# mttga/purejaxql

Measured on NVIDIA H100. Metric: MinAtar-Breakout env steps/sec @4096 envs x128 seeds, higher is better.
Workload: dtype f32

## Files before the change

### include/pqn_b200.h

```cpp
#ifndef PQN_B200_H
#define PQN_B200_H

#include <stdint.h>

#ifdef __cplusplus
extern "C" {
#endif

#define PQN_OK 0
#define PQN_E_INVALID (-1)
#define PQN_E_CUDA (-2)
#define PQN_E_UNSUPPORTED (-3)

#define PQN_ENV_BREAKOUT 0
#define PQN_ENV_ASTERIX 1
#define PQN_ENV_SPACE_INVADERS 2
#define PQN_ENV_FREEWAY 3
#define PQN_ENV_SEAQUEST 4
#define PQN_ENV_CARTPOLE 16
#define PQN_ENV_ACROBOT 17
#define PQN_ENV_MOUNTAIN_CAR 18
#define PQN_ENV_MEMORY_CHAIN 32
#define PQN_ENV_CATCH 33
#define PQN_ENV_DEEP_SEA 34
// ... 58 lines not shown
int pqn_rollout_act_step(int env_id, const uint32_t* step_keys, const float* q, const float* eps,
                         uint32_t* state, void* obs_next, int64_t obs_seed_stride, int32_t* action,
                         float* reward, uint8_t* done, float* maxq, int64_t tr_seed_stride, double* info_sums,
                         int info_done_only, int32_t S, int32_t E, int32_t env_total, int32_t env_offset, int max_steps,
                         float rew_scale, int rng_mode, void* stream);
int pqn_rollout_keys(uint32_t* rng_inout, uint32_t* keys_out, int32_t S, int32_t T, int rng_mode, void* stream);

int pqn_qlambda(const float* reward, const uint8_t* done, const float* maxq, const float* q_last,
                float* targets, int32_t T, int32_t S, int32_t E, int32_t A, float gamma, float lambda,
                void* stream);

#define PQN_NET_MINATAR_CNN 0
#define PQN_NET_MLP 1
#define PQN_NET_RNN 2
#define PQN_NET_MLP_BITS 3

typedef struct pqn_net_desc_t {
  int32_t kind;
  int32_t in_c;
  int32_t hidden;
  int32_t layers;
  int32_t num_actions;
  int32_t norm_type;
  int32_t norm_input;
} pqn_net_desc_t;
#define PQN_MAX_LAYERS 8
#define PQN_NORM_LAYER 0
#define PQN_NORM_BATCH 1
#define PQN_NORM_NONE 2

typedef struct pqn_net_layout_t {
  int64_t total;
  int64_t bn_scale, bn_bias;
  int64_t conv_w, conv_b;
  int64_t ln0_scale, ln0_bias;
  int64_t d0_w, d0_b;
  int64_t ln1_scale, ln1_bias;
  int64_t d1_w, d1_b;
  int64_t head_w, head_b;
  int64_t gru_ir_w, gru_ir_b, gru_iz_w, gru_iz_b, gru_in_w, gru_in_b, gru_hr_w, gru_hz_w, gru_hn_w, gru_hn_b;
} pqn_net_layout_t;

int pqn_net_layout(const pqn_net_desc_t* desc_host, pqn_net_layout_t* out_host);
int pqn_net_dense_layer(const pqn_net_desc_t* desc_host, int32_t layer, int64_t* offsets_host);
int64_t pqn_net_stats_floats(const pqn_net_desc_t* desc_host);
int64_t pqn_net_workspace_bytes(const pqn_net_desc_t* desc_host, int32_t S, int64_t rows);

int pqn_net_init(const pqn_net_desc_t* desc_host, const uint32_t* keys, float* params, int32_t S, void* stream);

int pqn_qnet_forward(const pqn_net_desc_t* desc_host, const float* params, const float* batch_stats, const void* obs,
                     const int32_t* gather, int64_t obs_rows_per_seed, float* q, int32_t S, int64_t rows,
                     void* workspace, void* stream);

int pqn_qnet_loss_grad(const pqn_net_desc_t* desc_host, const float* params, float* batch_stats, const void* obs,
                       const int32_t* gather, int64_t obs_rows_per_seed, const int32_t* action,
                       const float* target, int64_t tr_rows_per_seed, float* grads, float* loss_sum,
                       float* qsa_sum, float* bn_sums, int32_t S, int64_t rows, void* workspace, void* stream);

int pqn_rnn_step(const pqn_net_desc_t* desc_host, const float* params, float* hs, const float* obs,
                 int64_t obs_rows_per_seed, const uint8_t* last_done, const int32_t* last_action, float* q, int32_t S,
                 int32_t E, void* workspace, void* stream);
int pqn_rnn_loss_grad(const pqn_net_desc_t* desc_host, const float* params, const float* hs0, const float* obs,
                      const uint8_t* last_done, const int32_t* last_action, const int32_t* action, const float* reward,
                      const uint8_t* done, float* grads, float* loss_sum, float* qsa_sum, int32_t S, int32_t T, int32_t B,
                      float gamma, float lambda, void* workspace, void* stream);
int pqn_rnn_step_stats(const pqn_net_desc_t* desc_host, const float* params, const float* batch_stats, float* hs,
                       const float* obs, int64_t obs_rows_per_seed, const uint8_t* last_done, const int32_t* last_action,
                       float* q, int32_t S, int32_t E, void* workspace, void* stream);
int pqn_rnn_loss_grad_stats(const pqn_net_desc_t* desc_host, const float* params, float* batch_stats, const float* hs0,
                            const float* obs, const uint8_t* last_done, const int32_t* last_action,
                            const int32_t* action, const float* reward, const uint8_t* done, float* grads,
                            float* loss_sum, float* qsa_sum, int32_t S, int32_t T, int32_t B, float gamma, float lambda,
                            void* workspace, void* stream);

int pqn_radam_clip_step(float* params, const float* grads, float* mu, float* nu, const float* sched,
                        int32_t* step_counter, float* gnorm_scratch , int32_t S, int64_t P,
                        float max_norm, float b1, float b2, float eps, void* stream);

int pqn_bn_stats_update(float* batch_stats, float* bn_sums, int32_t S, int32_t F, int64_t stats_seed_stride,
                        float count, float momentum, void* stream);

int pqn_set_tensor_core_path(int on);
int pqn_set_conv_mma_path(int on);

int pqn_tc_split_lo(const float* x, float* lo, int64_t n, void* stream);
int pqn_tc_gemm_test(const float* a, const float* a_lo, const float* b, const float* b_lo, float* d, int32_t S,
                     int32_t M, int32_t N, int32_t K, int a_mn, int b_mn, int split3, void* stream);

int pqn_tc_split16(const float* x, void* hi, void* lo, int64_t n, float scale, void* stream);
int pqn_tc_gemm16_test(const void* a_hi, const void* a_lo, const void* b_hi, const void* b_lo, float* d, int32_t S,
                       int32_t M, int32_t N, int32_t K, int a_mn, int b_mn, float out_scale, void* stream);
int pqn_tc_dgrad16_test(const void* a_hi, const void* a_lo, const void* b_hi, const void* b_lo, const float* mask,
                        const uint32_t* relu_bits, float* d, int32_t S, int32_t M, int32_t N, int32_t K, int epi,
                        float out_scale, void* stream);

#ifdef __cplusplus
}
#endif
#endif
```

### purejaxql_b200/_lib.py

```python
from __future__ import annotations

import ctypes
import os
from ctypes import POINTER, Structure, c_char_p, c_double, c_float, c_int, c_int32, c_int64, c_longlong, c_void_p

HERE = os.path.dirname(os.path.abspath(__file__))
LIB_PATH = os.path.join(HERE, "libpqn_b200.so")


class EnvInfo(Structure):
    _fields_ = [("state_words", c_int32), ("obs_dim", c_int32), ("obs_shape", c_int32 * 3),
                ("num_actions", c_int32), ("max_steps", c_int32), ("binary_obs", c_int32),
                ("packed_obs_words", c_int32)]


class EnvParams(Structure):
    _fields_ = [("max_steps", c_int32), ("memory_length", c_int32)]


class NetDesc(Structure):
    _fields_ = [("kind", c_int32), ("in_c", c_int32), ("hidden", c_int32), ("layers", c_int32),
                ("num_actions", c_int32), ("norm_type", c_int32), ("norm_input", c_int32)]


NORM_TYPES = {"layer_norm": 0, "batch_norm": 1}


class NetLayout(Structure):
    _fields_ = [(n, c_int64) for n in (
        "total", "bn_scale", "bn_bias", "conv_w", "conv_b", "ln0_scale", "ln0_bias", "d0_w", "d0_b",
        "ln1_scale", "ln1_bias", "d1_w", "d1_b", "head_w", "head_b",
        "gru_ir_w", "gru_ir_b", "gru_iz_w", "gru_iz_b", "gru_in_w", "gru_in_b", "gru_hr_w", "gru_hz_w", "gru_hn_w",
        "gru_hn_b")]


class PqnError(RuntimeError):
    pass


_SIGS = {
    "pqn_last_error": (c_char_p, []),
    "pqn_version": (c_int, []),
    "pqn_launch_count": (c_longlong, []),
    "pqn_num_kernels": (c_int, []),
    "pqn_kernel_name": (c_char_p, [c_int]),
    "pqn_profile_enable": (c_int, [c_int]),
    "pqn_profile_read": (c_int, [POINTER(c_double), POINTER(c_longlong), c_int]),
    "pqn_env_info": (c_int, [c_int, POINTER(EnvInfo)]),
    "pqn_rng_split": (c_int, [c_void_p, c_int64, c_int32, c_void_p, c_int, c_void_p]),
    "pqn_threefry2x32": (c_int, [c_void_p, c_void_p, c_void_p, c_int64, c_void_p]),
    "pqn_rng_bits": (c_int, [c_void_p, c_int64, c_int64, c_void_p, c_int, c_void_p]),
    "pqn_random_normal": (c_int, [c_void_p, c_void_p, c_int64, c_int, c_void_p]),
    "pqn_normal_from_bits": (c_int, [c_void_p, c_void_p, c_int64, c_void_p]),
    "pqn_set_permutation_bucket_log2": (c_int, [c_int]),
    "pqn_permutation_workspace_bytes": (c_int64, [c_int64, c_int]),
    "pqn_permutation": (c_int, [c_void_p, c_int64, c_int, c_int, c_void_p, c_int64, c_void_p, c_void_p]),
    "pqn_env_reset": (c_int, [c_int, c_void_p, c_void_p, c_void_p, c_int64, c_int, c_int, c_void_p]),
    "pqn_env_reset_params": (c_int, [c_int, c_void_p, c_void_p, c_void_p, c_int64, POINTER(EnvParams), c_int, c_void_p]),
    "pqn_env_step": (c_int, [c_int, c_void_p, c_void_p, c_void_p, c_void_p, c_void_p, c_void_p, c_void_p,
                             c_void_p, c_void_p, c_void_p, c_int64, c_int, c_int, c_void_p]),
    "pqn_env_obs_packed": (c_int, [c_int, c_void_p, c_void_p, c_int64, c_void_p]),
    "pqn_env_obs": (c_int, [c_int, c_void_p, c_void_p, c_int64, c_void_p]),
    "pqn_eps_greedy": (c_int, [c_void_p, c_void_p, c_void_p, c_void_p, c_int64, c_int32, c_int, c_void_p]),
    "pqn_rollout_act_step": (c_int, [c_int, c_void_p, c_void_p, c_void_p, c_void_p, c_void_p, c_int64, c_void_p,
                                     c_void_p, c_void_p, c_void_p, c_int64, c_void_p, c_int, c_int32, c_int32,
                                     c_int32, c_int32, c_int, c_float, c_int, c_void_p]),
    "pqn_rollout_keys": (c_int, [c_void_p, c_void_p, c_int32, c_int32, c_int, c_void_p]),
    "pqn_qlambda": (c_int, [c_void_p, c_void_p, c_void_p, c_void_p, c_void_p, c_int32, c_int32, c_int32, c_int32,
                            c_float, c_float, c_void_p]),
    "pqn_net_layout": (c_int, [POINTER(NetDesc), POINTER(NetLayout)]),
    "pqn_net_dense_layer": (c_int, [POINTER(NetDesc), c_int32, POINTER(c_int64)]),
    "pqn_net_stats_floats": (c_int64, [POINTER(NetDesc)]),
    "pqn_net_workspace_bytes": (c_int64, [POINTER(NetDesc), c_int32, c_int64]),
    "pqn_net_init": (c_int, [POINTER(NetDesc), c_void_p, c_void_p, c_int32, c_void_p]),
    "pqn_qnet_forward": (c_int, [POINTER(NetDesc), c_void_p, c_void_p, c_void_p, c_void_p, c_int64, c_void_p, c_int32,
                                 c_int64, c_void_p, c_void_p]),
    "pqn_qnet_loss_grad": (c_int, [POINTER(NetDesc), c_void_p, c_void_p, c_void_p, c_void_p, c_int64, c_void_p,
                                   c_void_p, c_int64, c_void_p, c_void_p, c_void_p, c_void_p, c_int32, c_int64,
                                   c_void_p, c_void_p]),
    "pqn_rnn_step": (c_int, [POINTER(NetDesc), c_void_p, c_void_p, c_void_p, c_int64, c_void_p, c_void_p, c_void_p,
                             c_int32, c_int32, c_void_p, c_void_p]),
    "pqn_rnn_loss_grad": (c_int, [POINTER(NetDesc), c_void_p, c_void_p, c_void_p, c_void_p, c_void_p, c_void_p, c_void_p,
                                  c_void_p, c_void_p, c_void_p, c_void_p, c_int32, c_int32, c_int32, c_float, c_float,
                                  c_void_p, c_void_p]),
    "pqn_rnn_step_stats": (c_int, [POINTER(NetDesc), c_void_p, c_void_p, c_void_p, c_void_p, c_int64, c_void_p, c_void_p,
                                   c_void_p, c_int32, c_int32, c_void_p, c_void_p]),
    "pqn_rnn_loss_grad_stats": (c_int, [POINTER(NetDesc), c_void_p, c_void_p, c_void_p, c_void_p, c_void_p, c_void_p,
                                        c_void_p, c_void_p, c_void_p, c_void_p, c_void_p, c_void_p, c_int32, c_int32,
                                        c_int32, c_float, c_float, c_void_p, c_void_p]),
    "pqn_radam_clip_step": (c_int, [c_void_p, c_void_p, c_void_p, c_void_p, c_void_p, c_void_p, c_void_p, c_int32,
                                    c_int64, c_float, c_float, c_float, c_float, c_void_p]),
    "pqn_bn_stats_update": (c_int, [c_void_p, c_void_p, c_int32, c_int32, c_int64, c_float, c_float, c_void_p]),
    "pqn_set_tensor_core_path": (c_int, [c_int]),
    "pqn_set_conv_mma_path": (c_int, [c_int]),
    "pqn_tc_split_lo": (c_int, [c_void_p, c_void_p, c_int64, c_void_p]),
    "pqn_tc_split16": (c_int, [c_void_p, c_void_p, c_void_p, c_int64, c_float, c_void_p]),
    "pqn_tc_gemm_test": (c_int, [c_void_p, c_void_p, c_void_p, c_void_p, c_void_p, c_int32, c_int32, c_int32,
                                 c_int32, c_int, c_int, c_int, c_void_p]),
    "pqn_tc_gemm16_test": (c_int, [c_void_p, c_void_p, c_void_p, c_void_p, c_void_p, c_int32, c_int32, c_int32,
                                   c_int32, c_int, c_int, c_float, c_void_p]),
    "pqn_tc_dgrad16_test": (c_int, [c_void_p, c_void_p, c_void_p, c_void_p, c_void_p, c_void_p, c_void_p, c_int32,
                                    c_int32, c_int32, c_int32, c_int, c_float, c_void_p]),
}

EXPORTS = tuple(_SIGS)
_lib = None


def lib():
    global _lib
    if _lib is None:
        if not os.path.exists(LIB_PATH):
            raise PqnError(
                f"{LIB_PATH} is not built. Run `python -m purejaxql_b200.build` (needs nvcc). "
                "purejaxql_b200 has no CPU fallback.")
        l = ctypes.CDLL(LIB_PATH)
        for name, (res, args) in _SIGS.items():
            fn = getattr(l, name)
            fn.restype = res
            fn.argtypes = args
        _lib = l
    return _lib


def check(rc: int, what: str = ""):
    if rc != 0:
        msg = lib().pqn_last_error().decode("utf-8", "replace")
        raise PqnError(f"{what or 'libpqn_b200'} failed (rc={rc}): {msg}")


def p(t):
    if t is None:
        return None
    if not t.is_cuda:
        raise PqnError("libpqn_b200 takes CUDA tensors only (no CPU fallback); got a CPU tensor")
    if not t.is_contiguous():
        raise PqnError("libpqn_b200 takes contiguous tensors")
    return c_void_p(t.data_ptr())


def raw(t):
    if t is None:
        return None
    if not t.is_cuda:
        raise PqnError("libpqn_b200 takes CUDA tensors only (no CPU fallback); got a CPU tensor")
    return c_void_p(t.data_ptr())


def stream_ptr():
    import torch
    return c_void_p(torch.cuda.current_stream().cuda_stream)


def profile_read(reset=True):
    l = lib()
    n = l.pqn_num_kernels()
    ms = (c_double * n)()
    cnt = (c_longlong * n)()
    check(l.pqn_profile_read(ms, cnt, 1 if reset else 0), "pqn_profile_read")
    return {l.pqn_kernel_name(i).decode(): (ms[i], int(cnt[i])) for i in range(n) if cnt[i]}
```

### purejaxql_b200/csrc/pqn_net.cu

```cuda
#include <cuda_runtime.h>
#include <stdint.h>

#include "../../include/pqn_b200.h"
#include "api_common.h"
#include "tc_common.cuh"

namespace pqn {

constexpr int GT = 256;
constexpr int BK = 16;
constexpr float LN_EPS = 1e-6f;
constexpr int CONV_O = 16;
constexpr int CONV_PIX = 64;
constexpr int HID_CNN = 128;
constexpr int FLAT_CNN = CONV_PIX * CONV_O;

static int g_use_tc = 2;
static int g_conv_mma = 1;

__host__ __device__ static inline int64_t align4(int64_t x) { return (x + 3) & ~(int64_t)3; }

static int make_layout(const pqn_net_desc_t* d, pqn_net_layout_t* L) {
  int64_t off = 0;
  auto take = [&](int64_t n) { int64_t o = off; off += align4(n); return o; };
  L->d1_w = L->d1_b = L->ln1_scale = L->ln1_bias = L->conv_w = L->conv_b = -1;
  L->gru_ir_w = L->gru_ir_b = L->gru_iz_w = L->gru_iz_b = L->gru_in_w = L->gru_in_b = -1;
  L->gru_hr_w = L->gru_hz_w = L->gru_hn_w = L->gru_hn_b = -1;
  const int A = d->num_actions;
  const bool has_norm = d->norm_type != PQN_NORM_NONE;
  if (d->kind == PQN_NET_MINATAR_CNN) {
    const int C = d->in_c;
    L->bn_scale = take(C); L->bn_bias = take(C);
    L->conv_w = take(9 * C * CONV_O); L->conv_b = take(CONV_O);
    L->ln0_scale = L->ln0_bias = -1;
    if (has_norm) { L->ln0_scale = take(CONV_O); L->ln0_bias = take(CONV_O); }
    L->d0_w = take((int64_t)FLAT_CNN * HID_CNN); L->d0_b = take(HID_CNN);
    if (has_norm) { L->ln1_scale = take(HID_CNN); L->ln1_bias = take(HID_CNN); }
    L->head_w = take((int64_t)HID_CNN * A); L->head_b = take(A);
  } else if (d->kind == PQN_NET_MLP || d->kind == PQN_NET_RNN || d->kind == PQN_NET_MLP_BITS) {
    const int D = d->in_c, H = d->hidden;
    L->bn_scale = take(D); L->bn_bias = take(D);
    L->d0_w = take((int64_t)D * H); L->d0_b = take(H);
    L->ln0_scale = L->ln0_bias = -1;
    if (has_norm) { L->ln0_scale = take(H); L->ln0_bias = take(H); }
    for (int l = 1; l < d->layers; ++l) {
      const int64_t w = take((int64_t)H * H), b = take(H);
      const int64_t sc = has_norm ? take(H) : -1, bi = has_norm ? take(H) : -1;
      if (l == 1) { L->d1_w = w; L->d1_b = b; L->ln1_scale = sc; L->ln1_bias = bi; }
    }
    if (d->kind == PQN_NET_RNN) {
      L->gru_ir_w = take((int64_t)(H + A) * H); L->gru_ir_b = take(H);
      L->gru_iz_w = take((int64_t)(H + A) * H); L->gru_iz_b = take(H);
      L->gru_in_w = take((int64_t)(H + A) * H); L->gru_in_b = take(H);
      L->gru_hr_w = take((int64_t)H * H); L->gru_hz_w = take((int64_t)H * H);
      L->gru_hn_w = take((int64_t)H * H); L->gru_hn_b = take(H);
    }
    L->head_w = take((int64_t)H * A); L->head_b = take(A);
  } else {
    return -1;
  }
  L->total = off;
  return 0;
}

struct DenseOff { int64_t w, b, g, bi; };
__host__ __device__ inline DenseOff dense_off(const pqn_net_layout_t& L, int H, int l) {
  if (l == 0) return DenseOff{L.d0_w, L.d0_b, L.ln0_scale, L.ln0_bias};
  if (l == 1) return DenseOff{L.d1_w, L.d1_b, L.ln1_scale, L.ln1_bias};
  const bool norm = L.ln1_scale >= 0;
  const int64_t stride = align4((int64_t)H * H) + (norm ? 3 : 1) * align4(H);
  const int64_t w = (norm ? L.ln1_bias : L.d1_b) + align4(H) + (l - 2) * stride;
  const int64_t b = w + align4((int64_t)H * H);
  return DenseOff{w, b, norm ? b + align4(H) : -1, norm ? b + 2 * align4(H) : -1};
}

static int check_desc(const pqn_net_desc_t* d, const char* who) {
  if (!d) return set_error(PQN_E_INVALID, "%s: desc is NULL", who);
  if (d->num_actions < 1 || d->num_actions > 32) return set_error(PQN_E_INVALID, "%s: num_actions=%d out of [1,32]", who, d->num_actions);
  if (d->norm_type < 0 || d->norm_type > 2 || d->norm_input < 0 || d->norm_input > 1)
    return set_error(PQN_E_INVALID, "%s: norm_type=%d norm_input=%d", who, d->norm_type, d->norm_input);
  if (d->kind == PQN_NET_MLP || d->kind == PQN_NET_RNN || d->kind == PQN_NET_MLP_BITS) {
    const int H = d->hidden;
    if (H != 64 && H != 128 && H != 256 && H != 512)
      return set_error(PQN_E_UNSUPPORTED, "%s: hidden=%d (64, 128, 256 or 512 built)", who, H);
    if (d->layers < 1 || d->layers > PQN_MAX_LAYERS)
      return set_error(PQN_E_UNSUPPORTED, "%s: layers=%d (1 to %d built)", who, d->layers, PQN_MAX_LAYERS);
  }
  {
    const int Nh = d->kind == PQN_NET_MINATAR_CNN ? 128 : d->hidden;
    const size_t need = (size_t)(24 * Nh + 9 * d->num_actions * Nh + 8 * d->num_actions + 16) * sizeof(float);
    if (need > 227u * 1024u)
      return set_error(PQN_E_UNSUPPORTED, "%s: hidden=%d with num_actions=%d needs %zu B of shared memory for the head "
                       "backward (limit 227 KB)", who, Nh, d->num_actions, need);
  }
  if (d->kind == PQN_NET_MINATAR_CNN) {
    if (d->in_c != 4 && d->in_c != 6 && d->in_c != 7 && d->in_c != 10)
      return set_error(PQN_E_UNSUPPORTED, "%s: CNN in_c=%d (MinAtar uses 4/6/7/10)", who, d->in_c);
    return PQN_OK;
  }
  if (d->kind == PQN_NET_MLP_BITS) {
    if (d->in_c != 400 && d->in_c != 600 && d->in_c != 700)
// ... 494 lines not shown
      if (DZLO != nullptr) {
        float lo[V];
#pragma unroll
        for (int k = 0; k < V; ++k) lo[k] = tc::tf32_lo(dz[V * c + k]);
        st_feat<V>(DZLO + e, lo);
      }
    }
  }
#pragma unroll
  for (int j = 0; j < F; ++j) {
    const int f = (j / V) * CW + lane * V + (j % V);
    s_red3[warp * 3 * N + f] = a_dsc[j];
    s_red3[warp * 3 * N + N + f] = a_dbi[j];
    s_red3[warp * 3 * N + 2 * N + f] = a_db[j];
  }
  if (HEAD && lane == 0) { s_ls[warp * 2] = a_loss; s_ls[warp * 2 + 1] = a_qsa; }
  __syncthreads();
  const int stride = 3 * N + (HEAD ? A * N + A + 2 : 0);
  float* __restrict__ o = part + ((int64_t)seed * gridDim.x + blockIdx.x) * stride;
  for (int i = tid; i < 3 * N; i += 256) {
    float v = 0.f;
#pragma unroll
    for (int wv = 0; wv < 8; ++wv) v += s_red3[wv * 3 * N + i];
    o[i] = v;
  }
  if (HEAD) {
    for (int i = tid; i < A * N; i += 256) {
      float v = 0.f;
#pragma unroll
      for (int wv = 0; wv < 8; ++wv) v += s_dhw[wv * A * N + i];
      o[3 * N + i] = v;
    }
    if (tid < A + 2) {
      float v = 0.f;
      for (int wv = 0; wv < 8; ++wv) v += tid < A ? s_dhb[wv * A + tid] : s_ls[wv * 2 + (tid - A)];
      o[3 * N + A * N + tid] = v;
    }
  }
}

template <int SL>
__device__ __forceinline__ float ordered_partial_sum(const float* __restrict__ p, int count, int64_t stride, bool valid) {
  constexpr int COLS = 256 / SL;
  __shared__ float slice_sum[SL][COLS];
  const int col = threadIdx.x % COLS, sl = threadIdx.x / COLS;
  float v = 0.f;
  if (valid) {
#pragma unroll 4
    for (int c = sl; c < count; c += SL) v += p[(int64_t)c * stride];
  }
  slice_sum[sl][col] = v;
  __syncthreads();
  float r = 0.f;
  if (sl == 0) {
#pragma unroll
    for (int k = 0; k < SL; ++k) r += slice_sum[k][col];
  }
  return r;
}
static inline int final_slices(int count) { return count > 48 ? 32 : 8; }

template <int SL>
__global__ void row_bwd_final_kernel(const float* __restrict__ part, int nctas, int N, int A, int head,
                                     float* __restrict__ grads, int64_t P, int64_t off_dscale, int64_t off_dbias,
                                     int64_t off_db, int64_t off_hw, int64_t off_hb, float* __restrict__ loss_sum,
                                     float* __restrict__ qsa_sum) {
  const int seed = blockIdx.y;
  const int stride = 3 * N + (head ? A * N + A + 2 : 0);
  const int i = blockIdx.x * (256 / SL) + threadIdx.x % (256 / SL);
  const float v = ordered_partial_sum<SL>(part + (int64_t)seed * nctas * stride + i, nctas, stride, i < stride);
  if (i >= stride || threadIdx.x >= 256 / SL) return;
  float* __restrict__ g = grads + (int64_t)seed * P;
  if (i < N) g[off_dscale + i] = v;
  else if (i < 2 * N) g[off_dbias + (i - N)] = v;
  else if (i < 3 * N) g[off_db + (i - 2 * N)] = v;
  else if (i < 3 * N + A * N) {
    const int j = i - 3 * N, a = j / N, f = j - a * N;
    g[off_hw + (int64_t)f * A + a] = v;
  } else if (i < 3 * N + A * N + A) g[off_hb + (i - 3 * N - A * N)] = v;
  else if (i == 3 * N + A * N + A) loss_sum[seed] += v;
  else qsa_sum[seed] += v;
}

template <int C>
struct ConvCfg {
  static constexpr int TAPS = 9 * C;
  static constexpr int OBS_BITS = 100 * C;
  static constexpr int OBS_WORDS = (OBS_BITS + 31) / 32;
  static constexpr int PW = (OBS_WORDS + 3) / 4 * 4;
  static constexpr int SW = PW + 1;
};

template <int C>
__device__ __forceinline__ uint32_t pixel_bits(const uint32_t* __restrict__ so, int p) {
  const int f0 = p * C;
  const uint32_t lo = so[f0 >> 5], hi = so[(f0 >> 5) + 1];
  return __funnelshift_r(lo, hi, f0 & 31) & ((1u << C) - 1u);
}

template <int C>
__device__ __forceinline__ void conv_pixel(const uint32_t* __restrict__ so, const float* __restrict__ ws,
                                           const float* __restrict__ cb, int y, int x, float (&acc)[CONV_O]) {
#pragma unroll
  for (int o = 0; o < CONV_O; ++o) acc[o] = cb[o];
#pragma unroll
  for (int di = 0; di < 3; ++di)
#pragma unroll
    for (int dj = 0; dj < 3; ++dj) {
      const uint32_t nib = pixel_bits<C>(so, (y + di) * 10 + (x + dj));
      if (__ballot_sync(0xffffffffu, nib != 0u) == 0u) continue;
#pragma unroll
      for (int c = 0; c < C; ++c) {
        const bool bit = (nib >> c) & 1u;
        if (__ballot_sync(0xffffffffu, bit) == 0u) continue;
        const float* __restrict__ w = ws + ((di * 3 + dj) * C + c) * CONV_O;
#pragma unroll
        for (int o4 = 0; o4 < CONV_O / 4; ++o4) {
          const float4 wv = *reinterpret_cast<const float4*>(w + 4 * o4);
          if (bit) {
            acc[4 * o4] += wv.x; acc[4 * o4 + 1] += wv.y; acc[4 * o4 + 2] += wv.z; acc[4 * o4 + 3] += wv.w;
          }
        }
      }
    }
}

__device__ __forceinline__ void ln16(const float (&z)[CONV_O], float& mean, float& rstd) {
  float s1 = 0.f, s2 = 0.f;
#pragma unroll
  for (int o = 0; o < CONV_O; ++o) { s1 += z[o]; s2 = fmaf(z[o], z[o], s2); }
  mean = s1 * (1.0f / CONV_O);
  const float var = fmaxf(s2 * (1.0f / CONV_O) - mean * mean, 0.f);
  rstd = 1.0f / sqrtf(var + LN_EPS);
}

template <int C>
__device__ __forceinline__ void conv_load_consts(const float* __restrict__ prm, const pqn_net_layout_t& L, float* ws,
                                                 float* cb, float* sc, float* bi) {
  const float inv255 = 1.0f / 255.0f;
  for (int i = threadIdx.x; i < ConvCfg<C>::TAPS * CONV_O; i += blockDim.x) ws[i] = __ldg(prm + L.conv_w + i) * inv255;
  if (threadIdx.x < CONV_O) {
    cb[threadIdx.x] = __ldg(prm + L.conv_b + threadIdx.x);
    sc[threadIdx.x] = __ldg(prm + L.ln0_scale + threadIdx.x);
    bi[threadIdx.x] = __ldg(prm + L.ln0_bias + threadIdx.x);
  }
}

template <int C, bool TRAIN>
__global__ void __launch_bounds__(256) conv_fwd_kernel(const uint32_t* __restrict__ obs, int64_t obs_rows_per_seed,
                                                       const int32_t* __restrict__ gather,
                                                       const float* __restrict__ params, int64_t P,
                                                       pqn_net_layout_t L, float* __restrict__ H1,
                                                       float* __restrict__ H1LO, float* __restrict__ bn_sums,
                                                       int rows) {
  using Cfg = ConvCfg<C>;
  __shared__ __align__(16) float ws[Cfg::TAPS * CONV_O];
  __shared__ float cb[CONV_O], sc[CONV_O], bi[CONV_O];
  __shared__ uint32_t so[4][Cfg::SW];
  __shared__ float s_cnt[C];
  const int tid = threadIdx.x, sl = tid >> 6, pix = tid & 63;
  const int seed = blockIdx.y;
  const int row = blockIdx.x * 4 + sl;
  const bool valid = row < rows;
  conv_load_consts<C>(params + (int64_t)seed * P, L, ws, cb, sc, bi);
  if (TRAIN && tid < C) s_cnt[tid] = 0.f;
  if (pix < Cfg::SW) {
    uint32_t w = 0u;
    if (valid && pix < Cfg::PW) {
      const int64_t src = gather ? gather[(int64_t)seed * rows + row] : row;
      w = __ldg(obs + ((int64_t)seed * obs_rows_per_seed + src) * Cfg::PW + pix);
    }
    so[sl][pix] = w;
  }
  __syncthreads();
// ... 121 lines not shown
        float4 dz;
        dz.x = rstd * (dy[4 * o4] - m1 - acc[4 * o4] * m2);
        dz.y = rstd * (dy[4 * o4 + 1] - m1 - acc[4 * o4 + 1] * m2);
        dz.z = rstd * (dy[4 * o4 + 2] - m1 - acc[4 * o4 + 2] * m2);
        dz.w = rstd * (dy[4 * o4 + 3] - m1 - acc[4 * o4 + 3] * m2);
        *reinterpret_cast<float4*>(&my_dz[pix * SDZ_LD + 4 * o4]) = dz;
      }
    }
    __syncwarp();
#pragma unroll 8
    for (int p = tpar; p < CONV_PIX; p += 2) a_dcb += my_dz[p * SDZ_LD + o_b];
#pragma unroll
    for (int c = 0; c < C; ++c) {
      for (int wi = 0; wi < Cfg::OBS_WORDS; ++wi) {
        uint32_t bits = my_so[wi];
        if (C == 4) bits &= 0x11111111u << c;
        if (bits == 0u) continue;
        while (bits) {
          const int b = __ffs(bits) - 1;
          bits &= bits - 1u;
          const int f = wi * 32 + b;
          const int q = f / C;
          if (f - q * C != c) continue;
          const int qy = q / 10, qx = q - qy * 10;
#pragma unroll
          for (int it = 0; it < 5; ++it) {
            const int py = qy - t_di[it], px = qx - t_dj[it];
            if ((unsigned)py < 8u && (unsigned)px < 8u) wacc[c][it] += my_dz[(py * 8 + px) * SDZ_LD + o_b];
          }
        }
      }
    }
  }
  __syncthreads();
  for (int i = tid; i < TAPS * CONV_O; i += blockDim.x) s_w[i] = 0.f;
  __syncthreads();
  const float inv255 = 1.0f / 255.0f;
#pragma unroll
  for (int c = 0; c < C; ++c)
#pragma unroll
    for (int it = 0; it < 5; ++it) {
      const int tap = it * 2 + tpar;
      if (tap < 9) atomicAdd(&s_w[(tap * C + c) * CONV_O + o_b], wacc[c][it] * inv255);
    }
  atomicAdd(&s_red[2 * CONV_O + o_b], a_dcb);
#pragma unroll
  for (int o = 0; o < CONV_O; ++o) {
    float v0 = a_dsc[o], v1 = a_dbi[o];
#pragma unroll
    for (int sft = 16; sft > 0; sft >>= 1) {
      v0 += __shfl_xor_sync(0xffffffffu, v0, sft);
      v1 += __shfl_xor_sync(0xffffffffu, v1, sft);
    }
    if (lane == 0) {
      atomicAdd(&s_red[o], v0);
      atomicAdd(&s_red[CONV_O + o], v1);
    }
  }
  __syncthreads();
  float* __restrict__ g = grads + (int64_t)seed * P;
  for (int i = tid; i < TAPS * CONV_O; i += blockDim.x) atomicAdd(g + L.conv_w + i, s_w[i]);
  if (tid < CONV_O) {
    atomicAdd(g + L.ln0_scale + tid, s_red[tid]);
    atomicAdd(g + L.ln0_bias + tid, s_red[CONV_O + tid]);
    atomicAdd(g + L.conv_b + tid, s_red[2 * CONV_O + tid]);
  }
}

__device__ __forceinline__ void mma_tf32_16n8k8(float (&d)[4], const uint32_t (&a)[4], uint32_t b0, uint32_t b1) {
  asm volatile(
      "mma.sync.aligned.m16n8k8.row.col.f32.tf32.tf32.f32 {%0,%1,%2,%3}, {%4,%5,%6,%7}, {%8,%9}, {%0,%1,%2,%3};"
      : "+f"(d[0]), "+f"(d[1]), "+f"(d[2]), "+f"(d[3])
      : "r"(a[0]), "r"(a[1]), "r"(a[2]), "r"(a[3]), "r"(b0), "r"(b1));
}

template <int C>
struct ConvMma {
  static constexpr int TAPS = 9 * C;
  static constexpr int KS = (TAPS + 7) / 8;
  static constexpr int MT = (TAPS + 15) / 16;
};

template <int C>
struct PatchCfg {
  static constexpr int WORDS = (9 * C + 31) / 32;
};

template <int C>
__device__ __forceinline__ void patch_bits(const uint32_t* __restrict__ so, int pix, uint32_t (&w)[PatchCfg<C>::WORDS]) {
  constexpr int W = PatchCfg<C>::WORDS;
#pragma unroll
  for (int k = 0; k < W; ++k) w[k] = 0u;
  const int y = pix >> 3, x = pix & 7;
#pragma unroll
  for (int di = 0; di < 3; ++di) {
    const int f0 = ((y + di) * 10 + x) * C;
    const uint32_t r = __funnelshift_r(so[f0 >> 5], so[(f0 >> 5) + 1], f0 & 31) & ((1u << (3 * C)) - 1u);
    const int o = 3 * C * di;
    w[o >> 5] |= r << (o & 31);
    if ((o & 31) + 3 * C > 32) w[min((o >> 5) + 1, W - 1)] |= r >> (32 - (o & 31));
  }
}

template <int C>
__device__ __forceinline__ void build_patch(const uint32_t* __restrict__ so, int pix, uint32_t* __restrict__ out) {
  constexpr int W = PatchCfg<C>::WORDS;
  uint32_t w[W];
  patch_bits<C>(so, pix, w);
#pragma unroll
  for (int k = 0; k < W; ++k) out[k] = w[k];
}

template <int C>
__device__ __forceinline__ void build_patches(const uint32_t* __restrict__ so, uint32_t* __restrict__ patch, int lane) {
  build_patch<C>(so, lane, patch + lane * PatchCfg<C>::WORDS);
  build_patch<C>(so, lane + 32, patch + (lane + 32) * PatchCfg<C>::WORDS);
}

__device__ __forceinline__ uint32_t bit_f32(uint32_t word, int shift) {
  return ((word >> shift) & 1u) ? 0x3F800000u : 0u;
}

template <int C, bool EXPC = false>
__device__ __forceinline__ void conv_mma_load_weights(const float* __restrict__ prm, const pqn_net_layout_t& L,
                                                      float2* wb_hi, float2* wb_lo, float* cb, float* sc, float* bi) {
  using M = ConvMma<C>;
  const float inv255 = 1.0f / 255.0f;
  for (int i = threadIdx.x; i < M::KS * 2 * 32; i += blockDim.x) {
    const int ln = i & 31, h = (i >> 5) & 1, ks = i >> 6;
    const int o = h * 8 + (ln >> 2);
    const int t0 = ks * 8 + (ln & 3), t1 = t0 + 4;
    float w0 = t0 < M::TAPS ? __ldg(prm + L.conv_w + t0 * CONV_O + o) * inv255 : 0.f;
    float w1 = t1 < M::TAPS ? __ldg(prm + L.conv_w + t1 * CONV_O + o) * inv255 : 0.f;
    if (EXPC) {
      w0 *= __uint_as_float((254u - (1u << (t0 & 7))) << 23);
      w1 *= __uint_as_float((254u - (1u << (t1 & 7))) << 23);
    }
    const float h0 = __uint_as_float(__float_as_uint(w0) & 0xFFFFE000u), h1 = __uint_as_float(__float_as_uint(w1) & 0xFFFFE000u);
    wb_hi[i] = make_float2(h0, h1);
    wb_lo[i] = make_float2(w0 - h0, w1 - h1);
  }
  if (threadIdx.x < CONV_O) {
    cb[threadIdx.x] = __ldg(prm + L.conv_b + threadIdx.x);
    sc[threadIdx.x] = __ldg(prm + L.ln0_scale + threadIdx.x);
    bi[threadIdx.x] = __ldg(prm + L.ln0_bias + threadIdx.x);
  }
}

template <int C>
struct ExpPatch {
  static constexpr int KS = ConvMma<C>::KS;
  static constexpr int LD = KS | 1;
};

template <int C>
__device__ __forceinline__ void build_exp_patch(const uint32_t* __restrict__ so, int pix, uint32_t* __restrict__ out) {
  constexpr int W = PatchCfg<C>::WORDS;
  uint32_t w[W];
  patch_bits<C>(so, pix, w);
#pragma unroll
  for (int ks = 0; ks < ExpPatch<C>::KS; ++ks)
    out[ks] = ((w[(8 * ks) >> 5] >> ((8 * ks) & 31)) & 0xFFu) << 23;
}

template <int C>
__device__ __forceinline__ void conv_mma_block2_exp(const uint32_t* __restrict__ xp, const float2* __restrict__ wb_hi,
                                                    const float2* __restrict__ wb_lo, const float* __restrict__ cb,
                                                    int mbp, int lane, float (&z)[2][2][4]) {
  using E = ExpPatch<C>;
  const int g = lane >> 2, t = lane & 3;
  const uint32_t m_lo = 1u << (23 + t), m_hi = 1u << (27 + t);
#pragma unroll
  for (int i = 0; i < 2; ++i)
#pragma unroll
    for (int h = 0; h < 2; ++h) {
      z[i][h][0] = z[i][h][2] = cb[8 * h + 2 * t];
      z[i][h][1] = z[i][h][3] = cb[8 * h + 2 * t + 1];
    }
  const uint32_t* r00 = xp + (32 * mbp + g) * E::LD;
#pragma unroll
  for (int ks = 0; ks < E::KS; ++ks) {
    uint32_t a[2][4];
#pragma unroll
    for (int i = 0; i < 2; ++i) {
      const uint32_t w0 = r00[(16 * i) * E::LD + ks], w1 = r00[(16 * i + 8) * E::LD + ks];
      a[i][0] = w0 & m_lo; a[i][1] = w1 & m_lo; a[i][2] = w0 & m_hi; a[i][3] = w1 & m_hi;
    }
    float2 bl[2], bh[2];
#pragma unroll
    for (int h = 0; h < 2; ++h) {
      bl[h] = wb_lo[(ks * 2 + h) * 32 + lane];
      bh[h] = wb_hi[(ks * 2 + h) * 32 + lane];
    }
#pragma unroll
    for (int h = 0; h < 2; ++h)
#pragma unroll
      for (int i = 0; i < 2; ++i) mma_tf32_16n8k8(z[i][h], a[i], __float_as_uint(bl[h].x), __float_as_uint(bl[h].y));
#pragma unroll
    for (int h = 0; h < 2; ++h)
#pragma unroll
      for (int i = 0; i < 2; ++i) mma_tf32_16n8k8(z[i][h], a[i], __float_as_uint(bh[h].x), __float_as_uint(bh[h].y));
  }
}

__device__ __forceinline__ void ln16_quad(const float (&z)[2][4], float& mean0, float& rstd0, float& mean1,
                                          float& rstd1) {
  float s0 = z[0][0] + z[0][1] + z[1][0] + z[1][1];
  float q0 = z[0][0] * z[0][0] + z[0][1] * z[0][1] + z[1][0] * z[1][0] + z[1][1] * z[1][1];
  float s1 = z[0][2] + z[0][3] + z[1][2] + z[1][3];
  float q1 = z[0][2] * z[0][2] + z[0][3] * z[0][3] + z[1][2] * z[1][2] + z[1][3] * z[1][3];
#pragma unroll
  for (int o = 1; o <= 2; o <<= 1) {
    s0 += __shfl_xor_sync(0xffffffffu, s0, o); q0 += __shfl_xor_sync(0xffffffffu, q0, o);
    s1 += __shfl_xor_sync(0xffffffffu, s1, o); q1 += __shfl_xor_sync(0xffffffffu, q1, o);
  }
  mean0 = s0 * (1.0f / CONV_O); mean1 = s1 * (1.0f / CONV_O);
  rstd0 = rsqrtf(fmaxf(q0 * (1.0f / CONV_O) - mean0 * mean0, 0.f) + LN_EPS);
  rstd1 = rsqrtf(fmaxf(q1 * (1.0f / CONV_O) - mean1 * mean1, 0.f) + LN_EPS);
}

constexpr int CONV_MMA_WARPS = 8;

template <int C, bool TRAIN, bool H16 = false>
__global__ void __launch_bounds__(CONV_MMA_WARPS * 32, 3)
    conv_fwd_mma_kernel(const uint32_t* __restrict__ obs, int64_t obs_rows_per_seed, const int32_t* __restrict__ gather,
                        const float* __restrict__ params, int64_t P, pqn_net_layout_t L, float* __restrict__ H1,
                        float* __restrict__ H1LO, float* __restrict__ XH1, float* __restrict__ RS1,
                        uint32_t* __restrict__ RB, float* __restrict__ bn_sums, int rows) {
  using Cfg = ConvCfg<C>;
  using M = ConvMma<C>;
  __shared__ float2 wb_hi[M::KS * 2 * 32], wb_lo[M::KS * 2 * 32];
  __shared__ float cb[CONV_O], sc[CONV_O], bi[CONV_O];
  __shared__ uint32_t so[CONV_MMA_WARPS][Cfg::SW];
  __shared__ uint32_t sxp[CONV_MMA_WARPS][CONV_PIX * ExpPatch<C>::LD];
  __shared__ float s_cnt[C];
  const int tid = threadIdx.x, warp = tid >> 5, lane = tid & 31;
  const int g = lane >> 2, t = lane & 3;
  const int seed = blockIdx.y;
  conv_mma_load_weights<C, true>(params + (int64_t)seed * P, L, wb_hi, wb_lo, cb, sc, bi);
  if (TRAIN && tid < C) s_cnt[tid] = 0.f;
  __syncthreads();
  int cnt[C];
  uint32_t cmask[C];
#pragma unroll
  for (int c = 0; c < C; ++c) {
    cnt[c] = 0;
    cmask[c] = 0u;
    if (TRAIN) {
      for (int b = 0; b < 32; ++b) {
        const int f = lane * 32 + b;
        if (f < Cfg::OBS_BITS && f % C == c) cmask[c] |= 1u << b;
      }
    }
  }
  uint32_t* __restrict__ my_so = so[warp];
  static_assert(Cfg::PW <= 32, "one packed observation word per lane");
  if (lane == 0) my_so[Cfg::PW] = 0u;
  const int row_stride = gridDim.x * CONV_MMA_WARPS;
  auto fetch = [&](int r) -> uint32_t {
    if (r >= rows || lane >= Cfg::PW) return 0u;
    const int64_t src = gather ? gather[(int64_t)seed * rows + r] : r;
    return __ldg(obs + ((int64_t)seed * obs_rows_per_seed + src) * Cfg::PW + lane);
  };
  uint32_t pre = fetch(blockIdx.x * CONV_MMA_WARPS + warp);
  for (int row = blockIdx.x * CONV_MMA_WARPS + warp; row < rows; row += row_stride) {
    __syncwarp();
    if (lane < Cfg::PW) my_so[lane] = pre;
    if (TRAIN && bn_sums != nullptr) {
#pragma unroll
      for (int c = 0; c < C; ++c) cnt[c] += __popc(pre & cmask[c]);
    }
    __syncwarp();
    pre = fetch(row + row_stride);
    build_exp_patch<C>(my_so, lane, sxp[warp] + lane * ExpPatch<C>::LD);
    build_exp_patch<C>(my_so, lane + 32, sxp[warp] + (lane + 32) * ExpPatch<C>::LD);
    __syncwarp();
    float* __restrict__ hrow = H16 ? nullptr : H1 + ((int64_t)seed * rows + row) * FLAT_CNN;
    float* __restrict__ lrow = (!H16 && H1LO) ? H1LO + ((int64_t)seed * rows + row) * FLAT_CNN : nullptr;
    __half* __restrict__ hrow16 = H16 ? reinterpret_cast<__half*>(H1) + ((int64_t)seed * rows + row) * FLAT_CNN : nullptr;
    __half* __restrict__ lrow16 = H16 ? reinterpret_cast<__half*>(H1LO) + ((int64_t)seed * rows + row) * FLAT_CNN : nullptr;
    float* __restrict__ xrow = (TRAIN && XH1) ? XH1 + ((int64_t)seed * rows + row) * FLAT_CNN : nullptr;
    float* __restrict__ rrow = (TRAIN && RS1) ? RS1 + ((int64_t)seed * rows + row) * CONV_PIX : nullptr;
    uint16_t* __restrict__ brow =
        (TRAIN && RB) ? reinterpret_cast<uint16_t*>(RB + ((int64_t)seed * rows + row) * (FLAT_CNN / 32)) : nullptr;
#pragma unroll 1
    for (int mbp = 0; mbp < 2; ++mbp) {
     float z2[2][2][4];
     conv_mma_block2_exp<C>(sxp[warp], wb_hi, wb_lo, cb, mbp, lane, z2);
#pragma unroll
     for (int mi = 0; mi < 2; ++mi) {
      const int mb = 2 * mbp + mi;
      float (&z)[2][4] = z2[mi];
      float mean0, rstd0, mean1, rstd1;
      ln16_quad(z, mean0, rstd0, mean1, rstd1);
      uint32_t rb0 = 0u, rb1 = 0u;
#pragma unroll
      for (int h = 0; h < 2; ++h) {
        const int o = 8 * h + 2 * t;
        float2 v0, v1;
        v0.x = fmaxf((z[h][0] - mean0) * rstd0 * sc[o] + bi[o], 0.f);
        v0.y = fmaxf((z[h][1] - mean0) * rstd0 * sc[o + 1] + bi[o + 1], 0.f);
        v1.x = fmaxf((z[h][2] - mean1) * rstd1 * sc[o] + bi[o], 0.f);
        v1.y = fmaxf((z[h][3] - mean1) * rstd1 * sc[o + 1] + bi[o + 1], 0.f);
        const int p0 = 16 * mb + g, p1 = p0 + 8;
        if (H16) {
          __half2 h0, l0, h1v, l1;
          tc::split16x2<false>(fminf(v0.x, 65000.f), fminf(v0.y, 65000.f), h0, l0);
          tc::split16x2<false>(fminf(v1.x, 65000.f), fminf(v1.y, 65000.f), h1v, l1);
          *reinterpret_cast<__half2*>(hrow16 + p0 * CONV_O + o) = h0;
          *reinterpret_cast<__half2*>(lrow16 + p0 * CONV_O + o) = l0;
          *reinterpret_cast<__half2*>(hrow16 + p1 * CONV_O + o) = h1v;
          *reinterpret_cast<__half2*>(lrow16 + p1 * CONV_O + o) = l1;
        } else {
          *reinterpret_cast<float2*>(hrow + p0 * CONV_O + o) = v0;
          *reinterpret_cast<float2*>(hrow + p1 * CONV_O + o) = v1;
        }
        if (TRAIN) {
          rb0 |= ((v0.x > 0.f ? 1u : 0u) | (v0.y > 0.f ? 2u : 0u)) << o;
          rb1 |= ((v1.x > 0.f ? 1u : 0u) | (v1.y > 0.f ? 2u : 0u)) << o;
        }
        if (xrow) {
          *reinterpret_cast<float2*>(xrow + p0 * CONV_O + o) =
              make_float2((z[h][0] - mean0) * rstd0, (z[h][1] - mean0) * rstd0);
          *reinterpret_cast<float2*>(xrow + p1 * CONV_O + o) =
              make_float2((z[h][2] - mean1) * rstd1, (z[h][3] - mean1) * rstd1);
          if (h == 0 && t == 0) { rrow[p0] = rstd0; rrow[p1] = rstd1; }
        }
        if (lrow) {
          *reinterpret_cast<float2*>(lrow + p0 * CONV_O + o) = make_float2(tc::tf32_lo(v0.x), tc::tf32_lo(v0.y));
          *reinterpret_cast<float2*>(lrow + p1 * CONV_O + o) = make_float2(tc::tf32_lo(v1.x), tc::tf32_lo(v1.y));
        }
      }
      if (TRAIN && brow) {
        rb0 |= __shfl_xor_sync(0xffffffffu, rb0, 1); rb1 |= __shfl_xor_sync(0xffffffffu, rb1, 1);
        rb0 |= __shfl_xor_sync(0xffffffffu, rb0, 2); rb1 |= __shfl_xor_sync(0xffffffffu, rb1, 2);
        if (t == 0) { brow[16 * mb + g] = (uint16_t)rb0; brow[16 * mb + g + 8] = (uint16_t)rb1; }
      }
     }
    }
  }
  if (TRAIN && bn_sums != nullptr) {
#pragma unroll
    for (int c = 0; c < C; ++c) {
      int v = cnt[c];
#pragma unroll
      for (int o = 16; o > 0; o >>= 1) v += __shfl_xor_sync(0xffffffffu, v, o);
      if (lane == 0 && v) atomicAdd(&s_cnt[c], (float)v);
    }
    __syncthreads();
    if (tid < C && s_cnt[tid] != 0.f) {
      atomicAdd(bn_sums + (int64_t)seed * 2 * C + tid, s_cnt[tid]);
      atomicAdd(bn_sums + (int64_t)seed * 2 * C + C + tid, s_cnt[tid]);
    }
  }
}

__device__ __forceinline__ void mma_f16_16n8k16(float (&d)[4], const uint32_t (&a)[4], uint32_t b0, uint32_t b1) {
  asm volatile(
      "mma.sync.aligned.m16n8k16.row.col.f32.f16.f16.f32 {%0,%1,%2,%3}, {%4,%5,%6,%7}, {%8,%9}, {%0,%1,%2,%3};"
      : "+f"(d[0]), "+f"(d[1]), "+f"(d[2]), "+f"(d[3])
      : "r"(a[0]), "r"(a[1]), "r"(a[2]), "r"(a[3]), "r"(b0), "r"(b1));
}

template <int C>
struct Conv16 {
  static constexpr int TAPS = 9 * C;
  static constexpr int KS = (TAPS + 15) / 16;
  static constexpr int ROW = 2 * KS < 8 ? 8 : 2 * KS;
};

__host__ __device__ constexpr int conv16_channel(int h, int n) { return 4 * (n >> 1) + 2 * h + (n & 1); }

__host__ __device__ constexpr int conv16_tap(int s, int kk) {
  return 16 * s + (kk < 8 ? 0 : 8) + ((kk & 1) ? 4 : 0) + ((kk & 7) >> 1);
}

template <int C>
__device__ __forceinline__ void conv16_load_weights(const float* __restrict__ prm, const pqn_net_layout_t& L, uint4* wb,
                                                    float* cb, float* sc, float* bi) {
  using M = Conv16<C>;
  const float inv255 = 1.0f / 255.0f;
  for (int i = threadIdx.x; i < M::KS * 2 * 32; i += blockDim.x) {
    const int ln = i & 31, h = (i >> 5) & 1, s = i >> 6;
    const int gg = ln >> 2, tt = ln & 3;
    const int o = conv16_channel(h, gg);
    const float scale = __uint_as_float((uint32_t)(127 + 15 - (1 << tt)) << 23);
    float v[4];
#pragma unroll
    for (int q = 0; q < 4; ++q) {
      const int tap = conv16_tap(s, 2 * tt + (q & 1) + (q >> 1) * 8);
      v[q] = tap < M::TAPS ? __ldg(prm + L.conv_w + tap * CONV_O + o) * inv255 * scale : 0.f;
      v[q] = fminf(fmaxf(v[q], -65000.f), 65000.f);
    }
    const __half2 h0 = __floats2half2_rn(v[0], v[1]), h1 = __floats2half2_rn(v[2], v[3]);
    const float2 f0 = __half22float2(h0), f1 = __half22float2(h1);
    const __half2 l0 = __floats2half2_rn(v[0] - f0.x, v[1] - f0.y), l1 = __floats2half2_rn(v[2] - f1.x, v[3] - f1.y);
    wb[i] = make_uint4(*reinterpret_cast<const uint32_t*>(&h0), *reinterpret_cast<const uint32_t*>(&h1),
                       *reinterpret_cast<const uint32_t*>(&l0), *reinterpret_cast<const uint32_t*>(&l1));
  }
  if (threadIdx.x < CONV_O) {
    cb[threadIdx.x] = __ldg(prm + L.conv_b + threadIdx.x);
    sc[threadIdx.x] = __ldg(prm + L.ln0_scale + threadIdx.x);
    bi[threadIdx.x] = __ldg(prm + L.ln0_bias + threadIdx.x);
  }
}

template <int C>
__device__ __forceinline__ void build_patch16(const uint32_t* __restrict__ so, int pix, uint32_t* __restrict__ out) {
  constexpr int W = PatchCfg<C>::WORDS;
  uint32_t w[W];
  patch_bits<C>(so, pix, w);
#pragma unroll
  for (int b = 0; b < 2 * Conv16<C>::KS; ++b) {
    const int o = 8 * b;
    uint32_t v = (o >> 5) < W ? w[(o >> 5) < W ? (o >> 5) : 0] : 0u;
    const int sh = o & 31;
    const uint32_t lo = sh >= 10 ? v >> (sh - 10) : v << (10 - sh);
    const uint32_t hi = sh + 4 <= 26 ? v << (26 - sh - 4) : v >> (sh + 4 - 26);
    out[b] = __byte_perm(lo, hi, 0x7610);
  }
}

template <int C>
__device__ __forceinline__ void store_patch16(const uint32_t* __restrict__ so, int pix, uint32_t* __restrict__ row) {
  using M = Conv16<C>;
  uint32_t w[M::ROW];
#pragma unroll
  for (int k = 0; k < M::ROW; ++k) w[k] = 0u;
  build_patch16<C>(so, pix, w);
#pragma unroll
  for (int q = 0; q < M::ROW / 4; ++q)
    *reinterpret_cast<uint4*>(row + 4 * q) = make_uint4(w[4 * q], w[4 * q + 1], w[4 * q + 2], w[4 * q + 3]);
}

template <int C>
__device__ __forceinline__ void conv16_block2(const uint32_t* __restrict__ xp, const uint4* __restrict__ wb,
                                              const float* __restrict__ cb, int mbp, int lane, float (&z)[2][2][4]) {
  using M = Conv16<C>;
  const int g = lane >> 2, t = lane & 3;
  const uint32_t mask = (1u << (10 + t)) | (1u << (26 + t));
#pragma unroll
  for (int i = 0; i < 2; ++i)
#pragma unroll
    for (int h = 0; h < 2; ++h) {
      z[i][h][0] = z[i][h][2] = cb[4 * t + 2 * h];
      z[i][h][1] = z[i][h][3] = cb[4 * t + 2 * h + 1];
    }
  const uint32_t* r00 = xp + (32 * mbp + g) * M::ROW;
#pragma unroll
  for (int s = 0; s < M::KS; ++s) {
    uint32_t a[2][4];
#pragma unroll
    for (int i = 0; i < 2; ++i) {
      const uint2 w0 = *reinterpret_cast<const uint2*>(r00 + (16 * i) * M::ROW + 2 * s);
      const uint2 w1 = *reinterpret_cast<const uint2*>(r00 + (16 * i + 8) * M::ROW + 2 * s);
      a[i][0] = w0.x & mask; a[i][1] = w1.x & mask; a[i][2] = w0.y & mask; a[i][3] = w1.y & mask;
    }
    uint4 b[2];
#pragma unroll
    for (int h = 0; h < 2; ++h) b[h] = wb[(s * 2 + h) * 32 + lane];
#pragma unroll
    for (int h = 0; h < 2; ++h)
#pragma unroll
      for (int i = 0; i < 2; ++i) mma_f16_16n8k16(z[i][h], a[i], b[h].z, b[h].w);
#pragma unroll
    for (int h = 0; h < 2; ++h)
#pragma unroll
      for (int i = 0; i < 2; ++i) mma_f16_16n8k16(z[i][h], a[i], b[h].x, b[h].y);
  }
}

__device__ __forceinline__ uint32_t cvt_f16x2_satfinite(float lo, float hi) {
  uint32_t r;
  asm("cvt.rn.satfinite.f16x2.f32 %0, %1, %2;" : "=r"(r) : "f"(hi), "f"(lo));
  return r;
}

constexpr int CONV16_WARPS = 4;
constexpr int CONV16_CTAS_PER_SM = 5;

template <int C, bool TRAIN, bool H16>
__global__ void __launch_bounds__(CONV16_WARPS * 32, CONV16_CTAS_PER_SM)
    conv_fwd_mma16_kernel(const uint32_t* __restrict__ obs, int64_t obs_rows_per_seed, const int32_t* __restrict__ gather,
                          const float* __restrict__ params, int64_t P, pqn_net_layout_t L, float* __restrict__ H1,
                          float* __restrict__ H1LO, float* __restrict__ XH1, float* __restrict__ RS1,
                          uint32_t* __restrict__ RB, float* __restrict__ bn_sums, int rows) {
  using Cfg = ConvCfg<C>;
  using M = Conv16<C>;
  __shared__ __align__(16) uint4 wb[M::KS * 2 * 32];
  __shared__ float cb[CONV_O], sc[CONV_O], bi[CONV_O];
  __shared__ uint32_t so[CONV16_WARPS][Cfg::SW];
  __shared__ __align__(16) uint32_t sxp[CONV16_WARPS][CONV_PIX * M::ROW];
  __shared__ float s_cnt[C];
  const int tid = threadIdx.x, warp = tid >> 5, lane = tid & 31;
  const int g = lane >> 2, t = lane & 3;
  const int seed = blockIdx.y;
  conv16_load_weights<C>(params + (int64_t)seed * P, L, wb, cb, sc, bi);
  if (TRAIN && tid < C) s_cnt[tid] = 0.f;
  __syncthreads();
  int cnt[C];
  uint32_t cmask[C];
#pragma unroll
  for (int c = 0; c < C; ++c) {
    cnt[c] = 0;
    cmask[c] = 0u;
    if (TRAIN) {
      for (int b = 0; b < 32; ++b) {
        const int f = lane * 32 + b;
        if (f < Cfg::OBS_BITS && f % C == c) cmask[c] |= 1u << b;
      }
    }
  }
  uint32_t* __restrict__ my_so = so[warp];
  static_assert(Cfg::PW <= 32, "one packed observation word per lane");
  if (lane == 0) my_so[Cfg::PW] = 0u;
  const int row_stride = gridDim.x * CONV16_WARPS;
  auto fetch_index = [&](int r) -> int {
    const int rc = r < rows ? r : rows - 1;
    return gather ? __ldg(gather + (int64_t)seed * rows + rc) : rc;
  };
  auto fetch_obs = [&](int src) -> uint32_t {
    return __ldg(obs + ((int64_t)seed * obs_rows_per_seed + src) * Cfg::PW + (lane < Cfg::PW ? lane : 0));
  };
  const int row0 = blockIdx.x * CONV16_WARPS + warp;
  uint32_t pre = fetch_obs(fetch_index(row0));
  int src_next = fetch_index(row0 + row_stride);
  for (int row = row0; row < rows; row += row_stride) {
    __syncwarp();
    if (lane < Cfg::PW) my_so[lane] = pre;
    if (TRAIN && bn_sums != nullptr) {
#pragma unroll
      for (int c = 0; c < C; ++c) cnt[c] += __popc(pre & cmask[c]);
    }
    __syncwarp();
    pre = fetch_obs(src_next);
    src_next = fetch_index(row + 2 * row_stride);
    store_patch16<C>(my_so, lane, sxp[warp] + lane * M::ROW);
    store_patch16<C>(my_so, lane + 32, sxp[warp] + (lane + 32) * M::ROW);
    __syncwarp();
    const int64_t grow = (int64_t)seed * rows + row;
    float* __restrict__ hrow = H16 ? nullptr : H1 + grow * FLAT_CNN;
    __half* __restrict__ hrow16 = H16 ? reinterpret_cast<__half*>(H1) + grow * FLAT_CNN : nullptr;
    __half* __restrict__ lrow16 = H16 ? reinterpret_cast<__half*>(H1LO) + grow * FLAT_CNN : nullptr;
    float* __restrict__ xrow = (TRAIN && XH1) ? XH1 + grow * FLAT_CNN : nullptr;
    float* __restrict__ rrow = (TRAIN && RS1) ? RS1 + grow * CONV_PIX : nullptr;
    uint16_t* __restrict__ brow = (TRAIN && RB) ? reinterpret_cast<uint16_t*>(RB + grow * (FLAT_CNN / 32)) : nullptr;
    float keep_rs0 = 0.f, keep_rs1 = 0.f;
    uint32_t keep_rb = 0u;
#pragma unroll 1
    for (int mbp = 0; mbp < 2; ++mbp) {
      float z2[2][2][4];
      conv16_block2<C>(sxp[warp], wb, cb, mbp, lane, z2);
#pragma unroll
      for (int mi = 0; mi < 2; ++mi) {
        const int mb = 2 * mbp + mi;
        float (&z)[2][4] = z2[mi];
        float mean0, rstd0, mean1, rstd1;
        ln16_quad(z, mean0, rstd0, mean1, rstd1);
        const float nm0 = -mean0 * rstd0, nm1 = -mean1 * rstd1;
        uint32_t rb0 = 0u, rb1 = 0u;
        const int p0 = 16 * mb + g, p1 = p0 + 8, o4 = 4 * t;
        float x0[4], x1[4], v0[4], v1[4];
#pragma unroll
        for (int h = 0; h < 2; ++h) {
#pragma unroll
          for (int c = 0; c < 2; ++c) {
            const int o = o4 + 2 * h + c;
            x0[2 * h + c] = fmaf(z[h][c], rstd0, nm0);
            x1[2 * h + c] = fmaf(z[h][2 + c], rstd1, nm1);
            v0[2 * h + c] = fmaxf(fmaf(x0[2 * h + c], sc[o], bi[o]), 0.f);
            v1[2 * h + c] = fmaxf(fmaf(x1[2 * h + c], sc[o], bi[o]), 0.f);
          }
        }
        if (H16) {
          uint32_t hw0[2], hw1[2], lw0[2], lw1[2];
#pragma unroll
          for (int h = 0; h < 2; ++h) {
            hw0[h] = cvt_f16x2_satfinite(v0[2 * h], v0[2 * h + 1]);
            hw1[h] = cvt_f16x2_satfinite(v1[2 * h], v1[2 * h + 1]);
            const float2 f0 = __half22float2(*reinterpret_cast<const __half2*>(&hw0[h]));
// ... 922 lines not shown
  switch (C) {
    case 4: { LaunchScope _ls(TRAIN ? K_CONV_FWD : K_CONV_FWD_INFER, st); conv_fwd_kernel<4, TRAIN><<<grid, 256, 0, st>>>(obs, orps, gather, params, P, L, h1, h1lo, bn, rows); } break;
    case 6: { LaunchScope _ls(TRAIN ? K_CONV_FWD : K_CONV_FWD_INFER, st); conv_fwd_kernel<6, TRAIN><<<grid, 256, 0, st>>>(obs, orps, gather, params, P, L, h1, h1lo, bn, rows); } break;
    case 7: { LaunchScope _ls(TRAIN ? K_CONV_FWD : K_CONV_FWD_INFER, st); conv_fwd_kernel<7, TRAIN><<<grid, 256, 0, st>>>(obs, orps, gather, params, P, L, h1, h1lo, bn, rows); } break;
    case 10: { LaunchScope _ls(TRAIN ? K_CONV_FWD : K_CONV_FWD_INFER, st); conv_fwd_kernel<10, TRAIN><<<grid, 256, 0, st>>>(obs, orps, gather, params, P, L, h1, h1lo, bn, rows); } break;
    default: return -1;
  }
  return 0;
}

static unsigned conv_bwd_ctas(int S, int rows) {
  int per_seed = (device_sm_count() * 2 * 4 + S - 1) / S;
  const int maxc = (rows + CONV_BWD_WARPS - 1) / CONV_BWD_WARPS;
  if (per_seed > maxc) per_seed = maxc;
  if (per_seed < 1) per_seed = 1;
  return (unsigned)per_seed;
}

static int wgrad_splits(int tiles, int S, int rows) {
  int s = (2 * device_sm_count() + tiles * S - 1) / (tiles * S);
  const int maxs = (rows + 255) / 256;
  if (s > maxs) s = maxs;
  if (s < 1) s = 1;
  return s;
}

__global__ void split_lo_strided_kernel(const float* __restrict__ src, int64_t src_seed_stride, float* __restrict__ lo,
                                        int64_t n_per_seed) {
  const int seed = blockIdx.y;
  const int64_t i4 = (int64_t)blockIdx.x * blockDim.x + threadIdx.x;
  if (i4 * 4 >= n_per_seed) return;
  const float4 v = __ldg(reinterpret_cast<const float4*>(src + (int64_t)seed * src_seed_stride) + i4);
  reinterpret_cast<float4*>(lo + (int64_t)seed * n_per_seed)[i4] =
      make_float4(tc::tf32_lo(v.x), tc::tf32_lo(v.y), tc::tf32_lo(v.z), tc::tf32_lo(v.w));
}

static void launch_split_w1(const float* params, int64_t P, int64_t off_w, float* w1_lo, int S, cudaStream_t st) {
  const int64_t n = (int64_t)FLAT_CNN * HID_CNN;
  LaunchScope _ls(K_TC_SPLIT, st);
  split_lo_strided_kernel<<<dim3(cdiv(n / 4, 256), S), 256, 0, st>>>(params + off_w, P, w1_lo, n);
}

struct Planes16 { __half *h1_hi, *h1_lo, *dz_hi, *dz_lo, *w1_hi, *w1_lo; };
static Planes16 planes16(const Workspace& w, int S, int64_t rows) {
  const int64_t R = (int64_t)S * rows;
  Planes16 p;
  p.h1_hi = reinterpret_cast<__half*>(w.h1_lo); p.h1_lo = p.h1_hi + R * FLAT_CNN;
  p.dz_hi = reinterpret_cast<__half*>(w.dz2_lo); p.dz_lo = p.dz_hi + R * HID_CNN;
  p.w1_hi = reinterpret_cast<__half*>(w.w1_lo); p.w1_lo = p.w1_hi + (int64_t)S * FLAT_CNN * HID_CNN;
  return p;
}
static float grad_scale(int64_t rows) {
  float s = 16.f;
  while (rows > 1) { s *= 2.f; rows = (rows + 1) >> 1; }
  return s;
}

__global__ void split16_strided_kernel(const float* __restrict__ src, int64_t src_seed_stride, __half* __restrict__ hi,
                                       __half* __restrict__ lo, int64_t n_per_seed) {
  const int seed = blockIdx.y;
  const int64_t i4 = (int64_t)blockIdx.x * blockDim.x + threadIdx.x;
  if (i4 * 4 >= n_per_seed) return;
  const float4 v = __ldg(reinterpret_cast<const float4*>(src + (int64_t)seed * src_seed_stride) + i4);
  __half2 h0, h1, l0, l1;
  tc::split16x2(v.x, v.y, h0, l0);
  tc::split16x2(v.z, v.w, h1, l1);
  reinterpret_cast<uint2*>(hi + (int64_t)seed * n_per_seed)[i4] =
      make_uint2(*reinterpret_cast<uint32_t*>(&h0), *reinterpret_cast<uint32_t*>(&h1));
  reinterpret_cast<uint2*>(lo + (int64_t)seed * n_per_seed)[i4] =
      make_uint2(*reinterpret_cast<uint32_t*>(&l0), *reinterpret_cast<uint32_t*>(&l1));
}

static void launch_split16_w1(const float* params, int64_t P, int64_t off_w, const Planes16& pl, int S, cudaStream_t st) {
  const int64_t n = (int64_t)FLAT_CNN * HID_CNN;
  LaunchScope _ls(K_TC_SPLIT, st);
  split16_strided_kernel<<<dim3(cdiv(n / 4, 256), S), 256, 0, st>>>(params + off_w, P, pl.w1_hi, pl.w1_lo, n);
}
static void launch_split16_h1(const float* h1, const Planes16& pl, int64_t n, cudaStream_t st) {
  LaunchScope _ls(K_TC_SPLIT, st);
  split16_strided_kernel<<<dim3(cdiv(n / 4, 256), 1), 256, 0, st>>>(h1, 0, pl.h1_hi, pl.h1_lo, n);
}

static int tc16_dense_fwd(int epi, const float* params, int64_t P, const pqn_net_layout_t& L, const Workspace& w,
                          const Planes16& pl, int A, float* q, int S, int rows, cudaStream_t st) {
  CUtensorMap t[4];
  int rc;
  if ((rc = tc::make_tmap16(&t[0], pl.h1_hi, FLAT_CNN, rows, S, FLAT_CNN, (uint64_t)rows * FLAT_CNN, 128))) return rc;
  if ((rc = tc::make_tmap16(&t[1], pl.h1_lo, FLAT_CNN, rows, S, FLAT_CNN, (uint64_t)rows * FLAT_CNN, 128))) return rc;
  if ((rc = tc::make_tmap16(&t[2], pl.w1_hi, HID_CNN, FLAT_CNN, S, HID_CNN, (uint64_t)FLAT_CNN * HID_CNN, 64))) return rc;
  if ((rc = tc::make_tmap16(&t[3], pl.w1_lo, HID_CNN, FLAT_CNN, S, HID_CNN, (uint64_t)FLAT_CNN * HID_CNN, 64))) return rc;
  tc::GemmShape gs = {};
  gs.S = S; gs.M = rows; gs.m_tiles = (rows + 127) / 128; gs.n_tiles = 1; gs.k_blocks = FLAT_CNN / tc::TC_BK16;
  tc::EpiParams ep = {};
  ep.params = params; ep.P = P; ep.off_b = L.d0_b; ep.off_scale = L.ln1_scale; ep.off_bias = L.ln1_bias;
  ep.off_hw = L.head_w; ep.off_hb = L.head_b; ep.A = A; ep.rows = rows;
  ep.H = w.h2; ep.XHAT = w.xhat2; ep.RSTD = w.rstd2; ep.Q = q;
  return tc::launch_gemm16(0, 1, epi, t, gs, ep, st, epi == tc::EPI_LN_HEAD ? K_TC_FWD_HEAD : K_TC_FWD);
}

static int tc16_wgrad(float* grads, int64_t P, const pqn_net_layout_t& L, const Planes16& pl, int S, int rows,
                      float gscale, float* wg_part, cudaStream_t st) {
  CUtensorMap t[4];
  int rc;
  if ((rc = tc::make_tmap16(&t[0], pl.h1_hi, FLAT_CNN, rows, S, FLAT_CNN, (uint64_t)rows * FLAT_CNN, 64))) return rc;
  if ((rc = tc::make_tmap16(&t[1], pl.h1_lo, FLAT_CNN, rows, S, FLAT_CNN, (uint64_t)rows * FLAT_CNN, 64))) return rc;
  if ((rc = tc::make_tmap16(&t[2], pl.dz_hi, HID_CNN, rows, S, HID_CNN, (uint64_t)rows * HID_CNN, 64))) return rc;
  if ((rc = tc::make_tmap16(&t[3], pl.dz_lo, HID_CNN, rows, S, HID_CNN, (uint64_t)rows * HID_CNN, 64))) return rc;
  tc::GemmShape gs = {};
  gs.S = S; gs.M = FLAT_CNN; gs.m_tiles = FLAT_CNN / 128; gs.n_tiles = 1;
  gs.k_blocks = (rows + tc::TC_BK16 - 1) / tc::TC_BK16;
  gs.k_split = wgrad_ksplit(S * gs.m_tiles * gs.n_tiles, gs.k_blocks);
  tc::EpiParams ep = {};
  ep.ld_out = HID_CNN; ep.out_scale = 1.0f / gscale;
  const int64_t n = (int64_t)FLAT_CNN * HID_CNN;
  if (gs.k_split > 1) { ep.out = wg_part; ep.out_seed_stride = n; ep.split_stride = (int64_t)S * n; }
  else { ep.out = grads + L.d0_w; ep.out_seed_stride = P; }
  if ((rc = tc::launch_gemm16(1, 1, tc::EPI_STORE, t, gs, ep, st, K_TC_WGRAD))) return rc;
  if (gs.k_split > 1) {
    launch_split_reduce(wg_part, gs.k_split, (int64_t)S * n, n, S, grads + L.d0_w, P, st);
  }
  return 0;
}

static int tc16_dgrad(const Workspace& w, const Planes16& pl, int S, int rows, bool have_bits, float gscale,
                      cudaStream_t st) {
  CUtensorMap t[4];
  int rc;
  if ((rc = tc::make_tmap16(&t[0], pl.dz_hi, HID_CNN, rows, S, HID_CNN, (uint64_t)rows * HID_CNN, 128))) return rc;
  if ((rc = tc::make_tmap16(&t[1], pl.dz_lo, HID_CNN, rows, S, HID_CNN, (uint64_t)rows * HID_CNN, 128))) return rc;
  if ((rc = tc::make_tmap16(&t[2], pl.w1_hi, HID_CNN, FLAT_CNN, S, HID_CNN, (uint64_t)FLAT_CNN * HID_CNN, 128))) return rc;
  if ((rc = tc::make_tmap16(&t[3], pl.w1_lo, HID_CNN, FLAT_CNN, S, HID_CNN, (uint64_t)FLAT_CNN * HID_CNN, 128))) return rc;
  tc::GemmShape gs = {};
  gs.S = S; gs.M = rows; gs.m_tiles = (rows + 127) / 128; gs.n_tiles = FLAT_CNN / 128; gs.k_blocks = HID_CNN / tc::TC_BK16;
 
  tc::EpiParams ep = {};
  ep.out = w.h1; ep.mask = w.h1; ep.ld_out = FLAT_CNN; ep.out_seed_stride = (int64_t)rows * FLAT_CNN;
  ep.relu_bits = w.relu_bits; ep.rows = rows; ep.out_scale = 1.0f / gscale;
  return tc::launch_gemm16(0, 0, have_bits ? tc::EPI_RELU_BITS : tc::EPI_RELU_MASK, t, gs, ep, st, K_TC_DGRAD);
}

static int tc16_mm_store(const __half* a, int64_t a_plane, const __half* b, int64_t b_plane, float* out, int S, int rows, int K,
                         int N, cudaStream_t st, int kid) {
  CUtensorMap t[4];
  int rc;
  if ((rc = tc::make_tmap16(&t[0], a, K, rows, S, K, (uint64_t)rows * K, 128))) return rc;
  if ((rc = tc::make_tmap16(&t[1], a + a_plane, K, rows, S, K, (uint64_t)rows * K, 128))) return rc;
  if ((rc = tc::make_tmap16(&t[2], b, N, K, S, N, (uint64_t)K * N, 64))) return rc;
  if ((rc = tc::make_tmap16(&t[3], b + b_plane, N, K, S, N, (uint64_t)K * N, 64))) return rc;
  tc::GemmShape gs = {};
  gs.S = S; gs.M = rows; gs.m_tiles = (rows + 127) / 128; gs.n_tiles = N / 128; gs.k_blocks = (K + tc::TC_BK16 - 1) / tc::TC_BK16;
 
  tc::EpiParams ep = {};
  ep.out = out; ep.ld_out = N; ep.out_seed_stride = (int64_t)rows * N;
  return tc::launch_gemm16(0, 1, tc::EPI_STORE, t, gs, ep, st, kid);
}
static int tc16_mm_wgrad(const __half* a, int64_t a_plane, const __half* dz, int64_t dz_plane, float* out, int64_t out_seed_stride,
                         int S, int rows, int M, int N, float out_scale, float* wg_part, cudaStream_t st) {
  CUtensorMap t[4];
  int rc;
  if ((rc = tc::make_tmap16(&t[0], a, M, rows, S, M, (uint64_t)rows * M, 64))) return rc;
  if ((rc = tc::make_tmap16(&t[1], a + a_plane, M, rows, S, M, (uint64_t)rows * M, 64))) return rc;
  if ((rc = tc::make_tmap16(&t[2], dz, N, rows, S, N, (uint64_t)rows * N, 64))) return rc;
  if ((rc = tc::make_tmap16(&t[3], dz + dz_plane, N, rows, S, N, (uint64_t)rows * N, 64))) return rc;
  tc::GemmShape gs = {};
  gs.S = S; gs.M = M; gs.m_tiles = M / 128; gs.n_tiles = N / 128; gs.k_blocks = (rows + tc::TC_BK16 - 1) / tc::TC_BK16;
  gs.k_split = wgrad_ksplit(S * gs.m_tiles * gs.n_tiles, gs.k_blocks);
  tc::EpiParams ep = {};
  ep.ld_out = N; ep.out_scale = out_scale;
  const int64_t n = (int64_t)M * N;
  if (gs.k_split > 1) { ep.out = wg_part; ep.out_seed_stride = n; ep.split_stride = (int64_t)S * n; }
  else { ep.out = out; ep.out_seed_stride = out_seed_stride; }
  if ((rc = tc::launch_gemm16(1, 1, tc::EPI_STORE, t, gs, ep, st, K_TC_WGRAD))) return rc;
  if (gs.k_split > 1) {
    launch_split_reduce(wg_part, gs.k_split, (int64_t)S * n, n, S, out, out_seed_stride, st);
  }
  return 0;
}
static int tc16_mm_dgrad(const __half* dz, int64_t dz_plane, const __half* wgt, int64_t w_plane, const float* mask, float* out,
                         int S, int rows, int N, int Kp, float out_scale, cudaStream_t st) {
// ... 224 lines not shown
  if (rnn::modular_rnn(d)) {
    if ((rc = rnn::rnn_trunk_bwd_modular(d, L, params, obs, grads, S, rows, w, st))) return rc;
    return check_launch(who);
  }
  const dim3 rbg(conv_mma_ctas(S, rows, 4), S);
  float* dcur = w.dx;
  for (int l = d->layers - 1; l >= 0; --l) {
    const DenseOff o = dense_off(L, H, l);
    if ((rc = run_row_bwd(H, false, rbg, A, st, nullptr, w.xh[l], w.rs[l], dcur, dcur, nullptr, nullptr, nullptr, 1.0f, params,
                          grads, P, o.g, o.bi, o.b, 0, 0, nullptr, nullptr, nullptr, 0, nullptr, nullptr, w.rbp,
                          rows))) return rc;
    const float* xprev = l == 0 ? obs : w.h[l - 1];
    const int kin = l == 0 ? D : H;
    const int spl = wgrad_splits(ffma_tiles(kin, H), S, rows);
    run_wgrad_ffma(xprev, (int64_t)rows * kin, kin, dcur, (int64_t)rows * H, H, grads, P, o.w, rows, kin, S, spl, w.wgp, st);
    if (l > 0) {
      float* dnext = dcur == w.dhl ? w.dx : w.dhl;
      launch_dgrad(dcur, (int64_t)rows * H, H, params, P, o.w, w.h[l - 1], dnext, (int64_t)rows * H, rows, H, 0, S, st);
      dcur = dnext;
    }
  }
  return check_launch(who);
}

}

using namespace pqn;

extern "C" {

int64_t pqn_net_stats_floats(const pqn_net_desc_t* d) {
  if (check_desc(d, "pqn_net_stats_floats")) return -1;
  return nrm::stats_floats(d);
}

int pqn_rnn_step(const pqn_net_desc_t* d, const float* params, float* hs, const float* obs, int64_t obs_rows_per_seed,
                 const uint8_t* last_done, const int32_t* last_action, float* q, int32_t S, int32_t E, void* workspace,
                 void* stream) {
  int rc = check_desc(d, "pqn_rnn_step");
  if (rc) return rc;
  if ((rc = rnn::check_rnn(d, "pqn_rnn_step"))) return rc;
  return rnn_step(d, params, nullptr, hs, obs, obs_rows_per_seed, last_done, last_action, q, S, E, workspace, stream,
                  "pqn_rnn_step");
}

int pqn_rnn_step_stats(const pqn_net_desc_t* d, const float* params, const float* batch_stats, float* hs, const float* obs,
                       int64_t obs_rows_per_seed, const uint8_t* last_done, const int32_t* last_action, float* q, int32_t S,
                       int32_t E, void* workspace, void* stream) {
  int rc = check_desc(d, "pqn_rnn_step_stats");
  if (rc) return rc;
  if ((rc = rnn::check_rnn_stats(d, batch_stats, "pqn_rnn_step_stats"))) return rc;
  return rnn_step(d, params, batch_stats, hs, obs, obs_rows_per_seed, last_done, last_action, q, S, E, workspace, stream,
                  "pqn_rnn_step_stats");
}

int pqn_rnn_loss_grad(const pqn_net_desc_t* d, const float* params, const float* hs0, const float* obs,
                      const uint8_t* last_done, const int32_t* last_action, const int32_t* action, const float* reward,
                      const uint8_t* done, float* grads, float* loss_sum, float* qsa_sum, int32_t S, int32_t T, int32_t B,
                      float gamma, float lambda, void* workspace, void* stream) {
  int rc = check_desc(d, "pqn_rnn_loss_grad");
  if (rc) return rc;
  if ((rc = rnn::check_rnn(d, "pqn_rnn_loss_grad"))) return rc;
  return rnn_loss_grad(d, params, nullptr, hs0, obs, last_done, last_action, action, reward, done, grads, loss_sum, qsa_sum,
                       S, T, B, gamma, lambda, workspace, stream, "pqn_rnn_loss_grad");
}

int pqn_rnn_loss_grad_stats(const pqn_net_desc_t* d, const float* params, float* batch_stats, const float* hs0,
                            const float* obs, const uint8_t* last_done, const int32_t* last_action, const int32_t* action,
                            const float* reward, const uint8_t* done, float* grads, float* loss_sum, float* qsa_sum,
                            int32_t S, int32_t T, int32_t B, float gamma, float lambda, void* workspace, void* stream) {
  int rc = check_desc(d, "pqn_rnn_loss_grad_stats");
  if (rc) return rc;
  if ((rc = rnn::check_rnn_stats(d, batch_stats, "pqn_rnn_loss_grad_stats"))) return rc;
  return rnn_loss_grad(d, params, batch_stats, hs0, obs, last_done, last_action, action, reward, done, grads, loss_sum,
                       qsa_sum, S, T, B, gamma, lambda, workspace, stream, "pqn_rnn_loss_grad_stats");
}

int pqn_set_conv_mma_path(int on) {
  if (on != 0 && on != 1 && on != 3) return set_error(PQN_E_UNSUPPORTED, "pqn_set_conv_mma_path: no conv path %d", on);
  g_conv_mma = on;
  return PQN_OK;
}

int pqn_set_tensor_core_path(int on) {
  if (on < 0 || on > 2) return set_error(PQN_E_UNSUPPORTED, "pqn_set_tensor_core_path: no tensor-core path %d", on);
  g_use_tc = on;
  return PQN_OK;
}

int pqn_net_layout(const pqn_net_desc_t* d, pqn_net_layout_t* out) {
  int rc = check_desc(d, "pqn_net_layout");
  if (rc) return rc;
  if (!out) return set_error(PQN_E_INVALID, "pqn_net_layout: out is NULL");
  make_layout(d, out);
  return PQN_OK;
}

int pqn_net_dense_layer(const pqn_net_desc_t* d, int32_t layer, int64_t* offsets_host) {
  int rc = check_desc(d, "pqn_net_dense_layer");
  if (rc) return rc;
  if (d->kind != PQN_NET_MLP && d->kind != PQN_NET_RNN && d->kind != PQN_NET_MLP_BITS)
    return set_error(PQN_E_INVALID, "pqn_net_dense_layer: only the MLP and GRU networks have hidden dense layers");
  if (!offsets_host || layer < 0 || layer >= d->layers)
    return set_error(PQN_E_INVALID, "pqn_net_dense_layer: layer=%d out of [0,%d) or offsets NULL", layer, d->layers);
  pqn_net_layout_t L;
  make_layout(d, &L);
  const DenseOff o = dense_off(L, d->hidden, layer);
  offsets_host[0] = o.w; offsets_host[1] = o.b; offsets_host[2] = o.g; offsets_host[3] = o.bi;
  return PQN_OK;
}

int64_t pqn_net_workspace_bytes(const pqn_net_desc_t* d, int32_t S, int64_t rows) {
  if (check_desc(d, "pqn_net_workspace_bytes")) return -1;
  if (d->kind == PQN_NET_RNN) return rnn::carve_rnn(d, S, rows, nullptr, nullptr);
  if (modular_net(d)) return nrm::carve_norm(d, S, rows, nullptr, nullptr);
  return carve(d, S, rows, nullptr, nullptr) +
         (d->kind == PQN_NET_MLP_BITS ? bits::carve_bits(d, S, rows, nullptr, nullptr) : 0);
}

int pqn_qnet_forward(const pqn_net_desc_t* d, const float* params, const float* batch_stats, const void* obs,
                     const int32_t* gather, int64_t obs_rows_per_seed, float* q, int32_t S, int64_t rows, void* workspace,
                     void* stream) {
  int rc = check_desc(d, "pqn_qnet_forward");
  if (rc) return rc;
  if (!params || !obs || !q || !workspace || S <= 0 || rows <= 0 || S > 65535)
    return set_error(PQN_E_INVALID, "pqn_qnet_forward: bad argument");
  cudaStream_t st = (cudaStream_t)stream;
  pqn_net_layout_t L;
  make_layout(d, &L);
  if (modular_net(d)) {
    nrm::NormWs nw;
    nrm::carve_norm(d, S, rows, (char*)workspace, &nw);
    return nrm::norm_forward(d, L, params, const_cast<float*>(batch_stats), obs, gather, obs_rows_per_seed, q, S, (int)rows,
                            0, nullptr, nw, st);
  }
  Workspace w;
  carve(d, S, rows, (char*)workspace, &w);
  const int A = d->num_actions;
  if (d->kind == PQN_NET_MINATAR_CNN) {
    const bool use_tc = g_use_tc && A <= PQN_TC_MAX_A;
    const bool f16 = use_tc && g_use_tc == 2;
    const Planes16 pl = planes16(w, S, rows);
    const bool conv16 = f16 && g_conv_mma == 1;
    launch_conv_fwd<false>(d->in_c, dim3(cdiv(rows, 4), S), st, (const uint32_t*)obs, obs_rows_per_seed, gather, params,
                           L.total, L, conv16 ? (float*)pl.h1_hi : w.h1, conv16 ? (float*)pl.h1_lo : nullptr, nullptr,
                           (int)rows, nullptr, nullptr, nullptr, conv16);
    if (f16) {
      if (!conv16) launch_split16_h1(w.h1, pl, (int64_t)S * rows * FLAT_CNN, st);
      launch_split16_w1(params, L.total, L.d0_w, pl, S, st);
      if ((rc = tc16_dense_fwd(tc::EPI_LN_HEAD, params, L.total, L, w, pl, A, q, S, (int)rows, st))) return rc;
    } else if (use_tc) {
      launch_split_w1(params, L.total, L.d0_w, w.w1_lo, S, st);
      if ((rc = tc_dense_fwd(tc::EPI_LN_HEAD, params, L.total, L, w, A, q, S, (int)rows, st))) return rc;
    } else {
      if ((rc = launch_dense<2>(128, dim3(cdiv(rows, 128), S), st, w.h1, rows * FLAT_CNN, FLAT_CNN, params, L.total, L.d0_w,
                      L.d0_b, L.ln1_scale, L.ln1_bias, L.head_w, L.head_b, A, nullptr, nullptr, nullptr, q, (int)rows,
                      FLAT_CNN))) return rc;
    }
  } else {
    const int D = d->in_c, H = d->hidden;
    const bool bits = d->kind == PQN_NET_MLP_BITS, bits_tc = bits && g_use_tc == 2;
    const float* x = (const float*)obs;
    int64_t xss = obs_rows_per_seed * D;
    if (bits && !bits_tc) {
      bits::launch_expand((const uint32_t*)obs, obs_rows_per_seed, gather, (int)rows, D, w.xg, S, st);
      x = w.xg;
      xss = rows * D;
    } else if (gather && !bits) {
      { LaunchScope _ls(K_GATHER_ROWS, st); gather_rows_kernel<<<dim3(cdiv(rows * D, 256), S), 256, 0, st>>>(x, obs_rows_per_seed, gather, w.xg,
                                                                      (int)rows, D); }
      x = w.xg;
      xss = rows * D;
    }
    const int BM = (H == 128) ? 128 : 64;
    const dim3 grid(cdiv(rows, BM), S);
    const int last = d->layers - 1;
    if (bits_tc) {
      bits::BitsWs bw;
      bits::carve_bits(d, S, rows, (char*)workspace + carve(d, S, rows, nullptr, nullptr), &bw);
      if ((rc = bits_layer0_ln(d, L, params, (const uint32_t*)obs, obs_rows_per_seed, gather, S, (int)rows, w, bw, nullptr,
                               nullptr, st))) return rc;
      if (last == 0) {
        LaunchScope _ls(K_NORM_FWD, st);
        nrm::head_fwd_kernel<<<dim3(cdiv(rows, 8), S), 256, 0, st>>>(w.h[0], (int)rows, H, params, L.total, L.head_w, L.head_b, A, q);
      }
    } else if (last == 0) {
      if ((rc = dense_ln_fwd<2>(H, grid, st, x, xss, D, params, L.total, dense_off(L, H, 0), L.head_w, L.head_b, A, w.h[0], nullptr,
                      nullptr, q, (int)rows, D))) return rc;
    } else {
      if ((rc = dense_ln_fwd<0>(H, grid, st, x, xss, D, params, L.total, dense_off(L, H, 0), 0, 0, A, w.h[0], nullptr, nullptr, nullptr,
                      (int)rows, D))) return rc;
    }
    {
      for (int l = 1; l <= last; ++l) {
        if (mlp_hidden_tc(H)) {
          if ((rc = mlp_hidden_tc_fwd(w, L, params, L.total, H, l, S, (int)rows, nullptr, nullptr,
                                      l == last ? K_TC_FWD_HEAD : K_TC_FWD, st))) return rc;
          if (l == last) {
            LaunchScope _ls(K_NORM_FWD, st);
            nrm::head_fwd_kernel<<<dim3(cdiv(rows, 8), S), 256, 0, st>>>(w.h[l], (int)rows, H, params, L.total, L.head_w, L.head_b, A, q);
          }
        } else if (l == last) {
          if ((rc = dense_ln_fwd<2>(H, grid, st, w.h[l - 1], rows * H, H, params, L.total, dense_off(L, H, l), L.head_w, L.head_b, A,
                          w.h[l], nullptr, nullptr, q, (int)rows, H))) return rc;
        } else {
          if ((rc = dense_ln_fwd<0>(H, grid, st, w.h[l - 1], rows * H, H, params, L.total, dense_off(L, H, l), 0, 0, A, w.h[l], nullptr,
                          nullptr, nullptr, (int)rows, H))) return rc;
        }
      }
    }
  }
  return check_launch("pqn_qnet_forward");
}

int pqn_qnet_loss_grad(const pqn_net_desc_t* d, const float* params, float* batch_stats, const void* obs,
                       const int32_t* gather, int64_t obs_rows_per_seed, const int32_t* action, const float* target,
                       int64_t tr_rows_per_seed, float* grads, float* loss_sum, float* qsa_sum, float* bn_sums,
                       int32_t S, int64_t rows, void* workspace, void* stream) {
  int rc = check_desc(d, "pqn_qnet_loss_grad");
  if (rc) return rc;
  if (!params || !obs || !action || !target || !grads || !loss_sum || !qsa_sum || !workspace || S <= 0 || rows <= 0 ||
      S > 65535)
    return set_error(PQN_E_INVALID, "pqn_qnet_loss_grad: bad argument");
  cudaStream_t st = (cudaStream_t)stream;
  pqn_net_layout_t L;
  make_layout(d, &L);
// ... 152 lines not shown
```

### purejaxql_b200/csrc/pqn_tc.cu

```cuda
#include <cuda.h>
#include <cuda_runtime.h>
#include <stdint.h>

#include "../../include/pqn_b200.h"
#include "api_common.h"
#include "tc_common.cuh"

namespace pqn {
namespace tc {

constexpr int STG_LD = 36;

__device__ __forceinline__ void store_chunk_coalesced(float* stage, const float (&vals)[32], int lane, float* dst,
                                                      int64_t ld, int m_base, int M) {
#pragma unroll
  for (int j = 0; j < 8; ++j)
    *reinterpret_cast<float4*>(stage + lane * STG_LD + 4 * j) =
        make_float4(vals[4 * j], vals[4 * j + 1], vals[4 * j + 2], vals[4 * j + 3]);
  __syncwarp();
  const int r_in = lane >> 3, c4 = lane & 7;
#pragma unroll
  for (int it = 0; it < 8; ++it) {
    const int r = it * 4 + r_in;
    if (m_base + r < M)
      *reinterpret_cast<float4*>(dst + (int64_t)r * ld + 4 * c4) = *reinterpret_cast<const float4*>(stage + r * STG_LD + 4 * c4);
  }
  __syncwarp();
}

constexpr int SP_B = 0, SP_SC = 128, SP_BI = 256, SP_HW = 384 ,
              SP_HB = SP_HW + PQN_TC_MAX_A * 128, SP_FLOATS = SP_HB + PQN_TC_MAX_A;
static_assert(SP_FLOATS == TC_SP_FLOATS, "matches the TC_SMEM_BYTES budget in tc_common.cuh");

__device__ __forceinline__ void epi_bar_sync() { asm volatile("bar.sync 1, 128;" ::: "memory"); }
__device__ __forceinline__ void consumer_bar_sync() { asm volatile("bar.sync 2, 256;" ::: "memory"); }

template <int EPI>
__device__ __forceinline__ void stage_epi_params(const EpiParams& ep, float* sp, int seed, int et ) {
  const float* __restrict__ prm = ep.params + (int64_t)seed * ep.P;
  epi_bar_sync();
  sp[SP_B + et] = __ldg(prm + ep.off_b + et);
  sp[SP_SC + et] = __ldg(prm + ep.off_scale + et);
  sp[SP_BI + et] = __ldg(prm + ep.off_bias + et);
  if constexpr (EPI == EPI_LN_HEAD) {
    for (int a = 0; a < ep.A; ++a) sp[SP_HW + a * 128 + et] = __ldg(prm + ep.off_hw + (int64_t)et * ep.A + a);
    if (et < ep.A) sp[SP_HB + et] = __ldg(prm + ep.off_hb + et);
  }
  epi_bar_sync();
}

template <int EPI>
__device__ __forceinline__ void epilogue_ln_row(const EpiParams& ep, float (&acc)[128], float* stage, const float* sp,
                                                int lane, int seed, int m_base, int M) {
  const int m = m_base + lane;
  const bool row_ok = m < M;
  float s1 = 0.f, s2 = 0.f;
#pragma unroll
  for (int j4 = 0; j4 < 32; ++j4) {
    const float4 b = *reinterpret_cast<const float4*>(sp + SP_B + 4 * j4);
    const float bb[4] = {b.x, b.y, b.z, b.w};
#pragma unroll
    for (int e = 0; e < 4; ++e) {
      const int j = 4 * j4 + e;
      acc[j] += bb[e];
      s1 += acc[j];
      s2 = fmaf(acc[j], acc[j], s2);
    }
  }
  const float mean = s1 * (1.0f / 128.f);
  const float var = fmaxf(s2 * (1.0f / 128.f) - mean * mean, 0.f);
  const float rstd = 1.0f / sqrtf(var + 1e-6f);
  const int64_t grow = (int64_t)seed * ep.rows + m;
  if constexpr (EPI == EPI_LN_TRAIN) {
    float* hbase = ep.H + ((int64_t)seed * ep.rows + m_base) * 128;
    float* xbase = ep.XHAT + ((int64_t)seed * ep.rows + m_base) * 128;
#pragma unroll
    for (int c = 0; c < 4; ++c) {
      float xh[32], h[32];
#pragma unroll
      for (int j4 = 0; j4 < 8; ++j4) {
        const float4 s4 = *reinterpret_cast<const float4*>(sp + SP_SC + c * 32 + 4 * j4);
        const float4 b4 = *reinterpret_cast<const float4*>(sp + SP_BI + c * 32 + 4 * j4);
        const float ss[4] = {s4.x, s4.y, s4.z, s4.w}, bb[4] = {b4.x, b4.y, b4.z, b4.w};
#pragma unroll
        for (int e = 0; e < 4; ++e) {
          const int j = 4 * j4 + e;
          xh[j] = (acc[c * 32 + j] - mean) * rstd;
          h[j] = fmaxf(xh[j] * ss[e] + bb[e], 0.f);
        }
// ... 60 lines not shown
      for (int e = 0; e < 4; ++e) { mainacc[mi][ni][e] = 0.f; corr[mi][ni][e] = 0.f; }
  for (int kb = 0; kb < kbn; ++kb) {
    mbar_wait(&full[stage], phase);
    const uint8_t* sb = smem_al + stage * TC_STAGE_BYTES;
    if (kb % TC_PROMOTE == 0) {
#pragma unroll
      for (int mi = 0; mi < 2; ++mi)
#pragma unroll
        for (int ni = 0; ni < 8; ++ni)
#pragma unroll
          for (int e = 0; e < 4; ++e) mainacc[mi][ni][e] = 0.f;
    }
#pragma unroll
    for (int ks = 0; ks < TC_BK / 8; ++ks) {
      const int k = ks * 8 + tq;
      uint32_t ahi[2][4], alo[2][4];
#pragma unroll
      for (int mi = 0; mi < 2; ++mi) {
        const int r0 = wr + mi * 16 + g;
        const int rr[4] = {r0, r0 + 8, r0, r0 + 8}, kk[4] = {k, k, k + 4, k + 4};
#pragma unroll
        for (int e = 0; e < 4; ++e) {
          const float x = lds_tf32<A_MN>(sb + TC_A_HI, rr[e], kk[e]);
          ahi[mi][e] = tf32_trunc_bits(x);
          const float lo = split3 == 1 ? lds_tf32<A_MN>(sb + TC_A_LO, rr[e], kk[e]) : x - __uint_as_float(ahi[mi][e]);
          alo[mi][e] = tf32_trunc_bits(lo);
        }
      }
#pragma unroll
      for (int ni = 0; ni < 8; ++ni) {
        const int n = wc + ni * 8 + g;
        const uint32_t bh0 = tf32_trunc_bits(lds_tf32<B_MN>(sb + TC_B_HI, n, k));
        const uint32_t bh1 = tf32_trunc_bits(lds_tf32<B_MN>(sb + TC_B_HI, n, k + 4));
        if (split3) {
          const uint32_t bl0 = tf32_trunc_bits(lds_tf32<B_MN>(sb + TC_B_LO, n, k));
          const uint32_t bl1 = tf32_trunc_bits(lds_tf32<B_MN>(sb + TC_B_LO, n, k + 4));
#pragma unroll
          for (int mi = 0; mi < 2; ++mi) {
            mma_tf32_16x8x8(corr[mi][ni], alo[mi], bh0, bh1);
            mma_tf32_16x8x8(corr[mi][ni], ahi[mi], bl0, bl1);
          }
        }
#pragma unroll
        for (int mi = 0; mi < 2; ++mi) mma_tf32_16x8x8(mainacc[mi][ni], ahi[mi], bh0, bh1);
      }
    }
    __syncwarp();
    if (lane == 0) mbar_arrive(&empty[stage]);
    if (++stage == TC_STAGES) { stage = 0; phase ^= 1u; }
    if ((kb + 1) % TC_PROMOTE == 0 || kb == kbn - 1) {
      const bool first = kb < TC_PROMOTE;
#pragma unroll
      for (int mi = 0; mi < 2; ++mi)
#pragma unroll
        for (int ni = 0; ni < 8; ++ni)
#pragma unroll
          for (int h = 0; h < 2; ++h) {
            float2* p = reinterpret_cast<float2*>(tile_s + (wr + mi * 16 + g + 8 * h) * TC_ACC_LD + wc + ni * 8 + 2 * tq);
            const float2 v = make_float2(mainacc[mi][ni][2 * h], mainacc[mi][ni][2 * h + 1]);
            if (first) *p = v;
            else { const float2 o = *p; *p = make_float2(o.x + v.x, o.y + v.y); }
          }
    }
  }
#pragma unroll
  for (int mi = 0; mi < 2; ++mi)
#pragma unroll
    for (int ni = 0; ni < 8; ++ni)
#pragma unroll
      for (int h = 0; h < 2; ++h) {
        float2* p = reinterpret_cast<float2*>(tile_s + (wr + mi * 16 + g + 8 * h) * TC_ACC_LD + wc + ni * 8 + 2 * tq);
        float2 o = kbn > 0 ? *p : make_float2(0.f, 0.f);
        o.x += corr[mi][ni][2 * h];
        o.y += corr[mi][ni][2 * h + 1];
        *p = make_float2(o.x * osc, o.y * osc);
      }
}

template <int EPI, bool F16>
__host__ __device__ constexpr bool tma_store_epilogue() { return F16 && (EPI == EPI_RELU_MASK || EPI == EPI_RELU_BITS); }

__device__ __forceinline__ void wg_bar_sync(int wg) { asm volatile("bar.sync %0, 128;" ::"r"(3 + wg) : "memory"); }

template <int A_MN, int B_MN, int EPI, bool F16 = true>
__global__ void __launch_bounds__(TC_THREADS, 1)
    tc_gemm_kernel(const __grid_constant__ CUtensorMap tm_a_hi, const __grid_constant__ CUtensorMap tm_a_lo,
                   const __grid_constant__ CUtensorMap tm_b_hi, const __grid_constant__ CUtensorMap tm_b_lo,
                   const __grid_constant__ CUtensorMap tm_out, const GemmShape gs, const EpiParams ep) {
  constexpr bool TMA_EPI = tma_store_epilogue<EPI, F16>();
  extern __shared__ __align__(1024) uint8_t smem_raw[];
  const uint32_t smem_base = (smem_u32(smem_raw) + 1023u) & ~1023u;
  uint8_t* smem_al = smem_raw + (smem_base - smem_u32(smem_raw));
  float* tile_s = reinterpret_cast<float*>(smem_al + TC_STAGES * TC_STAGE_BYTES);
  float* sp_all = tile_s + 128 * TC_ACC_LD;
  uint64_t* full = reinterpret_cast<uint64_t*>(sp_all + TC_SP_FLOATS);
  uint64_t* empty = full + TC_STAGES;

  const int warp = threadIdx.x >> 5, lane = threadIdx.x & 31;

  if (warp == 8 && lane == 0) {
    prefetch_tmap(&tm_a_hi); prefetch_tmap(&tm_a_lo); prefetch_tmap(&tm_b_hi); prefetch_tmap(&tm_b_lo);
    if (TMA_EPI) prefetch_tmap(&tm_out);
    for (int i = 0; i < TC_STAGES; ++i) { mbar_init(&full[i], 1); mbar_init(&empty[i], TC_CONSUMERS / 32); }
    fence_barrier_init();
  }
  __syncthreads();

  const int ksplit = gs.k_split > 1 ? gs.k_split : 1;
  const int kb_per = (gs.k_blocks + ksplit - 1) / ksplit;
  const int tiles_per_seed = gs.m_tiles * gs.n_tiles * ksplit;
  const int num_tiles = tiles_per_seed * gs.S;
  auto decode = [&](int tile, int& seed, int& m0, int& n0, int& kb0, int& kbn) {
    seed = tile / tiles_per_seed;
    const int rem = tile - seed * tiles_per_seed;
    const int ks = rem % ksplit, mn = rem / ksplit;
    m0 = (mn / gs.n_tiles) * 128; n0 = (mn % gs.n_tiles) * 128;
    kb0 = ks * kb_per;
    kbn = min(kb_per, gs.k_blocks - kb0);
    if (kbn < 0) kbn = 0;
    return ks;
  };

  constexpr int BKE = F16 ? TC_BK16 : TC_BK;
  constexpr int MNB = F16 ? 2 : 4;
  constexpr int MNB_ELEMS = F16 ? 64 : 32, MNB_BYTES = F16 ? 8192 : 4096;
  const bool a_lo_tma = F16 || gs.split3 == 1, b_lo_tma = F16 || gs.split3 != 0;
  if (warp == 8) {
    if (lane == 0) {
      int stage = 0;
      uint32_t phase = 0;
      for (int tile = blockIdx.x; tile < num_tiles; tile += gridDim.x) {
        int seed, m0, n0, kb0, kbn;
        decode(tile, seed, m0, n0, kb0, kbn);
        for (int kb = kb0; kb < kb0 + kbn; ++kb) {
          mbar_wait(&empty[stage], phase ^ 1u);
          const uint32_t sb = smem_base + stage * TC_STAGE_BYTES;
          mbar_expect_tx(&full[stage], (2 + (a_lo_tma ? 1 : 0) + (b_lo_tma ? 1 : 0)) * TC_TILE_BYTES);
          const int k0 = kb * BKE;
          if (A_MN) {
#pragma unroll
            for (int j = 0; j < MNB; ++j) {
              tma_load_3d(sb + TC_A_HI + j * MNB_BYTES, &tm_a_hi, &full[stage], m0 + MNB_ELEMS * j, k0, seed);
              if (a_lo_tma) tma_load_3d(sb + TC_A_LO + j * MNB_BYTES, &tm_a_lo, &full[stage], m0 + MNB_ELEMS * j, k0, seed);
            }
          } else {
            tma_load_3d(sb + TC_A_HI, &tm_a_hi, &full[stage], k0, m0, seed);
            if (a_lo_tma) tma_load_3d(sb + TC_A_LO, &tm_a_lo, &full[stage], k0, m0, seed);
          }
          if (B_MN) {
#pragma unroll
            for (int j = 0; j < MNB; ++j) {
              tma_load_3d(sb + TC_B_HI + j * MNB_BYTES, &tm_b_hi, &full[stage], n0 + MNB_ELEMS * j, k0, seed);
              if (b_lo_tma) tma_load_3d(sb + TC_B_LO + j * MNB_BYTES, &tm_b_lo, &full[stage], n0 + MNB_ELEMS * j, k0, seed);
            }
          } else {
            tma_load_3d(sb + TC_B_HI, &tm_b_hi, &full[stage], k0, n0, seed);
            if (b_lo_tma) tma_load_3d(sb + TC_B_LO, &tm_b_lo, &full[stage], k0, n0, seed);
          }
          if (++stage == TC_STAGES) { stage = 0; phase ^= 1u; }
        }
      }
    }
    return;
  }

  const int t = threadIdx.x;
  const int wg = t >> 7;
  const uint32_t a_off = wg * 8192;
  const int fr = 64 * wg + 16 * ((t & 127) >> 5) + (lane >> 2), fc = 2 * (lane & 3);
  const int et = t & 127;
  uint8_t* out_stage = reinterpret_cast<uint8_t*>(tile_s) + wg * TC_OUT_STAGE_WG;
  int stage = 0;
  uint32_t phase = 0;
  for (int tile = blockIdx.x; tile < num_tiles; tile += gridDim.x) {
    int seed, m0, n0, kb0, kbn;
    const int ks_idx = decode(tile, seed, m0, n0, kb0, kbn);
    uint32_t rbits[2][4];
    if constexpr (TMA_EPI) {
      if constexpr (EPI == EPI_RELU_BITS) {
#pragma unroll
        for (int h = 0; h < 2; ++h) {
          const int m = m0 + fr + 8 * h;
          const uint4 w = m < gs.M ? __ldg(reinterpret_cast<const uint4*>(
                                         ep.relu_bits + ((int64_t)seed * ep.rows + m) * (ep.ld_out >> 5) + (n0 >> 5)))
                                   : make_uint4(0u, 0u, 0u, 0u);
          rbits[h][0] = w.x; rbits[h][1] = w.y; rbits[h][2] = w.z; rbits[h][3] = w.w;
        }
      } else {
        const int m = m0 + 64 * wg + (et >> 1);
// ... 116 lines not shown
          float2 o = kbn > 0 ? *p : make_float2(0.f, 0.f);
          if (kbn > 0) {
            o.x = fmaf(corr[4 * j + 2 * h], TC_LO_INV, o.x);
            o.y = fmaf(corr[4 * j + 2 * h + 1], TC_LO_INV, o.y);
          }
          *p = make_float2(o.x * osc, o.y * osc);
        }
    }
    }
    consumer_bar_sync();

    if constexpr (EPI == EPI_LN_TRAIN || EPI == EPI_LN_HEAD) {
      if (t < 128) {
        stage_epi_params<EPI>(ep, sp_all, seed, t);
        float acc[128];
        const float* row = tile_s + t * TC_ACC_LD;
#pragma unroll
        for (int j = 0; j < 32; ++j) {
          const float4 v = *reinterpret_cast<const float4*>(row + 4 * j);
          acc[4 * j] = v.x; acc[4 * j + 1] = v.y; acc[4 * j + 2] = v.z; acc[4 * j + 3] = v.w;
        }
        __syncwarp();
        epilogue_ln_row<EPI>(ep, acc, tile_s + warp * 32 * TC_ACC_LD, sp_all, lane, seed, m0 + warp * 32, gs.M);
      }
    } else {
      const int64_t base = (int64_t)seed * ep.out_seed_stride + n0;
      float* out = ep.out + (EPI == EPI_STORE ? (int64_t)ks_idx * ep.split_stride : 0) + base;
      for (int i = t; i < 128 * 32; i += TC_CONSUMERS) {
        const int r = i >> 5, c4 = i & 31, m = m0 + r;
        if (m >= gs.M) break;
        float4 v = *reinterpret_cast<const float4*>(tile_s + r * TC_ACC_LD + 4 * c4);
        if constexpr (EPI == EPI_RELU_MASK) {
          const float4 mk = *reinterpret_cast<const float4*>(ep.mask + base + (int64_t)m * ep.ld_out + 4 * c4);
          v.x = mk.x > 0.f ? v.x : 0.f; v.y = mk.y > 0.f ? v.y : 0.f;
          v.z = mk.z > 0.f ? v.z : 0.f; v.w = mk.w > 0.f ? v.w : 0.f;
        }
        if constexpr (EPI == EPI_RELU_BITS) {
          const uint32_t wd = __ldg(ep.relu_bits + ((int64_t)seed * ep.rows + m) * (ep.ld_out >> 5) + ((n0 >> 5) + (c4 >> 3)));
          const uint32_t b = wd >> (4 * (c4 & 7));
          v.x = (b & 1u) ? v.x : 0.f; v.y = (b & 2u) ? v.y : 0.f;
          v.z = (b & 4u) ? v.z : 0.f; v.w = (b & 8u) ? v.w : 0.f;
        }
        *reinterpret_cast<float4*>(out + (int64_t)m * ep.ld_out + 4 * c4) = v;
      }
    }
  }
  if constexpr (TMA_EPI) {
    if (et == 0) bulk_wait_all();
  }
}

typedef CUresult (*EncodeTiledFn)(CUtensorMap*, CUtensorMapDataType, cuuint32_t, void*, const cuuint64_t*,
                                  const cuuint64_t*, const cuuint32_t*, const cuuint32_t*, CUtensorMapInterleave,
                                  CUtensorMapSwizzle, CUtensorMapL2promotion, CUtensorMapFloatOOBfill);

static EncodeTiledFn get_encode() {
  static EncodeTiledFn fn = nullptr;
  if (!fn) {
    void* p = nullptr;
    cudaDriverEntryPointQueryResult qres;
    if (cudaGetDriverEntryPoint("cuTensorMapEncodeTiled", &p, cudaEnableDefault, &qres) != cudaSuccess || !p) return nullptr;
    fn = reinterpret_cast<EncodeTiledFn>(p);
  }
  return fn;
}

static int num_sms() { return device_sm_count(); }

int make_tmap(CUtensorMap* tm, const float* base, uint64_t inner, uint64_t mid, uint64_t seeds, uint64_t mid_stride_elems,
              uint64_t seed_stride_elems, uint32_t box_mid) {
  EncodeTiledFn enc = get_encode();
  if (!enc) return set_error(PQN_E_CUDA, "cuTensorMapEncodeTiled entry point unavailable");
  cuuint64_t dims[3] = {inner, mid, seeds};
  cuuint64_t strides[2] = {mid_stride_elems * 4, seed_stride_elems * 4};
  cuuint32_t box[3] = {32, box_mid, 1};
  cuuint32_t estr[3] = {1, 1, 1};
  CUresult r = enc(tm, CU_TENSOR_MAP_DATA_TYPE_FLOAT32, 3, const_cast<float*>(base), dims, strides, box, estr,
                   CU_TENSOR_MAP_INTERLEAVE_NONE, CU_TENSOR_MAP_SWIZZLE_128B, CU_TENSOR_MAP_L2_PROMOTION_L2_256B,
                   CU_TENSOR_MAP_FLOAT_OOB_FILL_NONE);
  if (r != CUDA_SUCCESS) return set_error(PQN_E_CUDA, "cuTensorMapEncodeTiled failed (%d)", (int)r);
  return PQN_OK;
}

template <int A_MN, int B_MN, int EPI, bool F16>
static int launch_t(const CUtensorMap* t, const GemmShape& gs, const EpiParams& ep, cudaStream_t st, int kid) {
  auto kfn = tc_gemm_kernel<A_MN, B_MN, EPI, F16>;
  static_assert(TC_SMEM_BYTES <= 227 * 1024, "dynamic shared memory of the GEMM kernel exceeds the per-CTA limit");
  if (cudaFuncSetAttribute(kfn, cudaFuncAttributeMaxDynamicSharedMemorySize, TC_SMEM_BYTES) != cudaSuccess)
    return check_launch("tc_gemm(cudaFuncSetAttribute)");
  CUtensorMap tm_out = t[0];
  if (tma_store_epilogue<EPI, F16>()) {
    if (ep.ld_out != (int64_t)gs.n_tiles * 128 || gs.k_split > 1)
      return set_error(PQN_E_INVALID, "tc_gemm16: ReLU-mask epilogues need ld_out == N and no split-K");
    int rc = make_tmap(&tm_out, ep.out, (uint64_t)ep.ld_out, (uint64_t)gs.M, (uint64_t)gs.S, (uint64_t)ep.ld_out,
                       (uint64_t)ep.out_seed_stride, 64);
    if (rc) return rc;
  }
  const int tiles = gs.m_tiles * gs.n_tiles * gs.S * (gs.k_split > 1 ? gs.k_split : 1);
  const int grid = tiles < num_sms() ? tiles : num_sms();
  {
    LaunchScope _ls(kid < 0 ? (int)K_TC_GEMM : kid, st);
    kfn<<<grid, TC_THREADS, TC_SMEM_BYTES, st>>>(t[0], t[1], t[2], t[3], tm_out, gs, ep);
  }
  return check_launch("tc_gemm");
}

int launch_gemm(int a_mn, int b_mn, int epi, const CUtensorMap* t, const GemmShape& gs, const EpiParams& ep,
                cudaStream_t st, int kernel_id) {
#define PQN_TC_CASE(A, B, E) \
  if (a_mn == A && b_mn == B && epi == E) return launch_t<A, B, E, false>(t, gs, ep, st, kernel_id);
  PQN_TC_CASE(0, 1, EPI_STORE)
  PQN_TC_CASE(0, 1, EPI_LN_TRAIN)
  PQN_TC_CASE(0, 1, EPI_LN_HEAD)
  PQN_TC_CASE(1, 1, EPI_STORE)
  PQN_TC_CASE(0, 0, EPI_STORE)
  PQN_TC_CASE(0, 0, EPI_RELU_MASK)
  PQN_TC_CASE(0, 0, EPI_RELU_BITS)
#undef PQN_TC_CASE
  return set_error(PQN_E_UNSUPPORTED, "tc_gemm: combination a_mn=%d b_mn=%d epi=%d not instantiated", a_mn, b_mn, epi);
}

int launch_gemm16(int a_mn, int b_mn, int epi, const CUtensorMap* t, const GemmShape& gs, const EpiParams& ep,
                  cudaStream_t st, int kernel_id) {
#define PQN_TC_CASE(A, B, E) \
  if (a_mn == A && b_mn == B && epi == E) return launch_t<A, B, E, true>(t, gs, ep, st, kernel_id);
  PQN_TC_CASE(0, 1, EPI_STORE)
  PQN_TC_CASE(0, 1, EPI_LN_TRAIN)
  PQN_TC_CASE(0, 1, EPI_LN_HEAD)
  PQN_TC_CASE(1, 1, EPI_STORE)
  PQN_TC_CASE(0, 0, EPI_STORE)
  PQN_TC_CASE(0, 0, EPI_RELU_MASK)
  PQN_TC_CASE(0, 0, EPI_RELU_BITS)
#undef PQN_TC_CASE
  return set_error(PQN_E_UNSUPPORTED, "tc_gemm16: combination a_mn=%d b_mn=%d epi=%d not instantiated", a_mn, b_mn, epi);
}

int make_tmap16(CUtensorMap* tm, const void* base, uint64_t inner, uint64_t mid, uint64_t seeds, uint64_t mid_stride_elems,
                uint64_t seed_stride_elems, uint32_t box_mid) {
  EncodeTiledFn enc = get_encode();
  if (!enc) return set_error(PQN_E_CUDA, "cuTensorMapEncodeTiled entry point unavailable");
  cuuint64_t dims[3] = {inner, mid, seeds};
  cuuint64_t strides[2] = {mid_stride_elems * 2, seed_stride_elems * 2};
  cuuint32_t box[3] = {64, box_mid, 1};
  cuuint32_t estr[3] = {1, 1, 1};
  CUresult r = enc(tm, CU_TENSOR_MAP_DATA_TYPE_FLOAT16, 3, const_cast<void*>(base), dims, strides, box, estr,
                   CU_TENSOR_MAP_INTERLEAVE_NONE, CU_TENSOR_MAP_SWIZZLE_128B, CU_TENSOR_MAP_L2_PROMOTION_L2_256B,
                   CU_TENSOR_MAP_FLOAT_OOB_FILL_NONE);
  if (r != CUDA_SUCCESS) return set_error(PQN_E_CUDA, "cuTensorMapEncodeTiled(fp16) failed (%d)", (int)r);
  return PQN_OK;
}

__global__ void split_lo_kernel(const float* __restrict__ x, float* __restrict__ lo, int64_t n4) {
  const int64_t i = (int64_t)blockIdx.x * blockDim.x + threadIdx.x;
  if (i >= n4) return;
  const float4 v = __ldg(reinterpret_cast<const float4*>(x) + i);
  float4 o;
  o.x = tf32_lo(v.x); o.y = tf32_lo(v.y); o.z = tf32_lo(v.z); o.w = tf32_lo(v.w);
  reinterpret_cast<float4*>(lo)[i] = o;
}

__global__ void split16_kernel(const float* __restrict__ x, __half* __restrict__ hi, __half* __restrict__ lo, int64_t n4,
                               float scale) {
  const int64_t i = (int64_t)blockIdx.x * blockDim.x + threadIdx.x;
  if (i >= n4) return;
  const float4 v = __ldg(reinterpret_cast<const float4*>(x) + i);
  __half2 h0, h1, l0, l1;
  split16x2(v.x * scale, v.y * scale, h0, l0);
  split16x2(v.z * scale, v.w * scale, h1, l1);
  reinterpret_cast<uint2*>(hi)[i] = make_uint2(*reinterpret_cast<uint32_t*>(&h0), *reinterpret_cast<uint32_t*>(&h1));
  reinterpret_cast<uint2*>(lo)[i] = make_uint2(*reinterpret_cast<uint32_t*>(&l0), *reinterpret_cast<uint32_t*>(&l1));
}

}
}

using namespace pqn;
using namespace pqn::tc;

extern "C" {

int pqn_tc_split_lo(const float* x, float* lo, int64_t n, void* stream) {
  if (!x || !lo || n < 0 || (n & 3)) return set_error(PQN_E_INVALID, "pqn_tc_split_lo: bad argument (n %% 4 == 0)");
  if (n == 0) return PQN_OK;
  {
    LaunchScope _ls(K_TC_SPLIT, (cudaStream_t)stream);
    split_lo_kernel<<<(unsigned)((n / 4 + 255) / 256), 256, 0, (cudaStream_t)stream>>>(x, lo, n / 4);
  }
  return check_launch("pqn_tc_split_lo");
}

int pqn_tc_split16(const float* x, void* hi, void* lo, int64_t n, float scale, void* stream) {
  if (!x || !hi || !lo || n < 0 || (n & 3)) return set_error(PQN_E_INVALID, "pqn_tc_split16: bad argument (n %% 4 == 0)");
  if (n == 0) return PQN_OK;
  {
    LaunchScope _ls(K_TC_SPLIT, (cudaStream_t)stream);
    split16_kernel<<<(unsigned)((n / 4 + 255) / 256), 256, 0, (cudaStream_t)stream>>>(x, (__half*)hi, (__half*)lo, n / 4,
                                                                                       scale);
  }
  return check_launch("pqn_tc_split16");
}

int pqn_tc_gemm16_test(const void* a_hi, const void* a_lo, const void* b_hi, const void* b_lo, float* d, int32_t S,
                       int32_t M, int32_t N, int32_t K, int a_mn, int b_mn, float out_scale, void* stream) {
  if (!a_hi || !a_lo || !b_hi || !b_lo || !d || S <= 0 || M <= 0 || N <= 0 || K <= 0 || (N % 128) || (K % 8) || (M % 8))
    return set_error(PQN_E_INVALID, "pqn_tc_gemm16_test: bad argument");
  CUtensorMap t[4];
  int rc;
  const void* ap[2] = {a_hi, a_lo};
  const void* bp[2] = {b_hi, b_lo};
  for (int i = 0; i < 2; ++i) {
    if (a_mn) { if ((rc = make_tmap16(&t[i], ap[i], M, K, S, M, (uint64_t)M * K, 64))) return rc; }
    else { if ((rc = make_tmap16(&t[i], ap[i], K, M, S, K, (uint64_t)M * K, 128))) return rc; }
    if (b_mn) { if ((rc = make_tmap16(&t[2 + i], bp[i], N, K, S, N, (uint64_t)N * K, 64))) return rc; }
    else { if ((rc = make_tmap16(&t[2 + i], bp[i], K, N, S, K, (uint64_t)N * K, 128))) return rc; }
  }
  GemmShape gs = {};
  gs.S = S; gs.M = M; gs.m_tiles = (M + 127) / 128; gs.n_tiles = N / 128; gs.k_blocks = (K + TC_BK16 - 1) / TC_BK16;
// ... 54 lines not shown
```

### purejaxql_b200/csrc/tc_common.cuh

```cuda
#pragma once
#include <cuda.h>
#include <cuda_fp16.h>
#include <stdint.h>

namespace pqn {
namespace tc {

constexpr int TC_CONSUMERS = 256;
constexpr int TC_THREADS = TC_CONSUMERS + 32;
constexpr int TC_BK16 = 64;
constexpr int TC_BK = 32;
constexpr int TC_STAGES = 2;
constexpr int TC_PROMOTE = 4;
constexpr int TC_TILE_BYTES = 128 * TC_BK16 * 2;
constexpr float TC_LO_SCALE = 2048.0f, TC_LO_INV = 1.0f / 2048.0f;
constexpr int TC_A_HI = 0, TC_A_LO = TC_TILE_BYTES, TC_B_HI = 2 * TC_TILE_BYTES, TC_B_LO = 3 * TC_TILE_BYTES;
constexpr int TC_STAGE_BYTES = 4 * TC_TILE_BYTES;
constexpr int TC_ACC_LD = 132;
constexpr int TC_SP_FLOATS = 384 + 8 * 128 + 8;
constexpr int TC_SMEM_BYTES = TC_STAGES * TC_STAGE_BYTES + 128 * TC_ACC_LD * 4 + TC_SP_FLOATS * 4 + 256  +
                              1024 ;
constexpr int TC_OUT_BOX_BYTES = 64 * 32 * 4;
constexpr int TC_OUT_STAGE_WG = 34 * 1024;
static_assert(TC_OUT_STAGE_WG >= 64 * TC_ACC_LD * 4 && TC_OUT_STAGE_WG + 4 * TC_OUT_BOX_BYTES <= 128 * TC_ACC_LD * 4,
              "each warpgroup's output staging lies within its own 64 rows of the fp32 tile, 1024-byte aligned");
#define PQN_TC_MAX_A 8

enum Epilogue : int { EPI_STORE = 0, EPI_LN_TRAIN = 1, EPI_LN_HEAD = 2, EPI_RELU_MASK = 3, EPI_RELU_BITS = 4 };

struct GemmShape {
  int S;
  int M;
  int m_tiles, n_tiles, k_blocks;
  int split3;
  int k_split;
};

struct EpiParams {
  int64_t split_stride;
  float out_scale;
  float* out;
  const float* mask;
  const uint32_t* relu_bits;
  int64_t ld_out, out_seed_stride;
  const float* params;
  int64_t P, off_b, off_scale, off_bias, off_hw, off_hb;
  int A, rows;
  float *H, *XHAT, *RSTD, *Q;
};

__device__ __forceinline__ uint32_t smem_u32(const void* p) { return (uint32_t)__cvta_generic_to_shared(p); }

__device__ __forceinline__ float tf32_lo(float x) {
  const float hi = __uint_as_float(__float_as_uint(x) & 0xFFFFE000u);
  return x - hi;
}

__device__ __forceinline__ void mbar_init(uint64_t* bar, int count) {
  asm volatile("mbarrier.init.shared::cta.b64 [%0], %1;" ::"r"(smem_u32(bar)), "r"(count) : "memory");
}
__device__ __forceinline__ void fence_barrier_init() { asm volatile("fence.mbarrier_init.release.cluster;" ::: "memory"); }
__device__ __forceinline__ void mbar_expect_tx(uint64_t* bar, uint32_t bytes) {
  asm volatile("mbarrier.arrive.expect_tx.shared::cta.b64 _, [%0], %1;" ::"r"(smem_u32(bar)), "r"(bytes) : "memory");
}
__device__ __forceinline__ void mbar_arrive(uint64_t* bar) {
  asm volatile("mbarrier.arrive.shared::cta.b64 _, [%0];" ::"r"(smem_u32(bar)) : "memory");
}
__device__ __forceinline__ void mbar_wait(uint64_t* bar, uint32_t parity) {
  const uint32_t addr = smem_u32(bar);
  uint32_t ok;
  do {
    asm volatile(
        "{\n\t.reg .pred p;\n\t"
        "mbarrier.try_wait.parity.shared::cta.b64 p, [%1], %2;\n\t"
        "selp.u32 %0, 1, 0, p;\n\t}"
        : "=r"(ok)
        : "r"(addr), "r"(parity)
        : "memory");
  } while (!ok);
}

__device__ __forceinline__ void prefetch_tmap(const CUtensorMap* tm) {
  asm volatile("prefetch.tensormap [%0];" ::"l"(reinterpret_cast<uint64_t>(tm)) : "memory");
}
__device__ __forceinline__ void tma_load_3d(uint32_t smem_dst, const CUtensorMap* tm, uint64_t* bar, int c0, int c1, int c2) {
  asm volatile(
      "cp.async.bulk.tensor.3d.shared::cluster.global.mbarrier::complete_tx::bytes [%0], [%1, {%3, %4, %5}], [%2];"
      ::"r"(smem_dst), "l"(reinterpret_cast<uint64_t>(tm)), "r"(smem_u32(bar)), "r"(c0), "r"(c1), "r"(c2)
      : "memory");
}
__device__ __forceinline__ void tma_store_3d(const CUtensorMap* tm, uint32_t smem_src, int c0, int c1, int c2) {
  asm volatile("cp.async.bulk.tensor.3d.global.shared::cta.bulk_group [%0, {%2, %3, %4}], [%1];"
               ::"l"(reinterpret_cast<uint64_t>(tm)), "r"(smem_src), "r"(c0), "r"(c1), "r"(c2)
               : "memory");
}
__device__ __forceinline__ void bulk_commit() { asm volatile("cp.async.bulk.commit_group;" ::: "memory"); }
__device__ __forceinline__ void bulk_wait_read_all() { asm volatile("cp.async.bulk.wait_group.read 0;" ::: "memory"); }
__device__ __forceinline__ void bulk_wait_all() { asm volatile("cp.async.bulk.wait_group 0;" ::: "memory"); }
__device__ __forceinline__ void fence_proxy_async_smem() { asm volatile("fence.proxy.async.shared::cta;" ::: "memory"); }

__device__ __forceinline__ void wgmma_fence() { asm volatile("wgmma.fence.sync.aligned;" ::: "memory"); }
__device__ __forceinline__ void wgmma_commit() { asm volatile("wgmma.commit_group.sync.aligned;" ::: "memory"); }
template <int N>
__device__ __forceinline__ void wgmma_wait() { asm volatile("wgmma.wait_group.sync.aligned %0;" ::"n"(N) : "memory"); }
__device__ __forceinline__ void fence_operands(float (&d)[64]) {
#pragma unroll
  for (int i = 0; i < 64; ++i) asm volatile("" : "+f"(d[i])::"memory");
}

template <int TA, int TB>
__device__ __forceinline__ void wgmma_f16_m64n128(float (&d)[64], uint64_t desc_a, uint64_t desc_b, uint32_t scale_d) {
  asm volatile(
      "{\n\t.reg .pred p;\n\t"
      "setp.ne.b32 p, %66, 0;\n\t"
      "wgmma.mma_async.sync.aligned.m64n128k16.f32.f16.f16 "
      "{%0, %1, %2, %3, %4, %5, %6, %7, %8, %9, %10, %11, %12, %13, %14, %15, %16, %17, %18, %19, %20, %21, %22, %23, "
      "%24, %25, %26, %27, %28, %29, %30, %31, %32, %33, %34, %35, %36, %37, %38, %39, %40, %41, %42, %43, %44, %45, "
      "%46, %47, %48, %49, %50, %51, %52, %53, %54, %55, %56, %57, %58, %59, %60, %61, %62, %63}, "
      "%64, %65, p, 1, 1, %67, %68;\n\t}"
      : "+f"(d[0]), "+f"(d[1]), "+f"(d[2]), "+f"(d[3]), "+f"(d[4]), "+f"(d[5]), "+f"(d[6]), "+f"(d[7]), "+f"(d[8]),
        "+f"(d[9]), "+f"(d[10]), "+f"(d[11]), "+f"(d[12]), "+f"(d[13]), "+f"(d[14]), "+f"(d[15]), "+f"(d[16]),
        "+f"(d[17]), "+f"(d[18]), "+f"(d[19]), "+f"(d[20]), "+f"(d[21]), "+f"(d[22]), "+f"(d[23]), "+f"(d[24]),
        "+f"(d[25]), "+f"(d[26]), "+f"(d[27]), "+f"(d[28]), "+f"(d[29]), "+f"(d[30]), "+f"(d[31]), "+f"(d[32]),
        "+f"(d[33]), "+f"(d[34]), "+f"(d[35]), "+f"(d[36]), "+f"(d[37]), "+f"(d[38]), "+f"(d[39]), "+f"(d[40]),
        "+f"(d[41]), "+f"(d[42]), "+f"(d[43]), "+f"(d[44]), "+f"(d[45]), "+f"(d[46]), "+f"(d[47]), "+f"(d[48]),
        "+f"(d[49]), "+f"(d[50]), "+f"(d[51]), "+f"(d[52]), "+f"(d[53]), "+f"(d[54]), "+f"(d[55]), "+f"(d[56]),
        "+f"(d[57]), "+f"(d[58]), "+f"(d[59]), "+f"(d[60]), "+f"(d[61]), "+f"(d[62]), "+f"(d[63])
      : "l"(desc_a), "l"(desc_b), "r"(scale_d), "n"(TA), "n"(TB));
}

template <int MN>
__device__ __forceinline__ uint64_t make_gdesc16(uint32_t tile_addr, int ks) {
  const uint32_t addr = MN ? tile_addr + ks * 2048 : tile_addr + ks * 32;
  const uint64_t lbo = MN ? (8192u >> 4) : 1u;
  const uint64_t sbo = 1024u >> 4;
  return (uint64_t)((addr >> 4) & 0x3FFFu) | (lbo << 16) | (sbo << 32) | (1ull << 62);
}

__device__ __forceinline__ void split16(float x, __half& hi, __half& lo) {
  x = fminf(fmaxf(x, -65000.0f), 65000.0f);
  hi = __float2half_rn(x);
  lo = __float2half_rn((x - __half2float(hi)) * TC_LO_SCALE);
}
template <bool SAT = true>
__device__ __forceinline__ void split16x2(float x0, float x1, __half2& hi, __half2& lo) {
  if (SAT) {
    x0 = fminf(fmaxf(x0, -65000.0f), 65000.0f);
    x1 = fminf(fmaxf(x1, -65000.0f), 65000.0f);
  }
  hi = __floats2half2_rn(x0, x1);
  const float2 hf = __half22float2(hi);
  lo = __floats2half2_rn((x0 - hf.x) * TC_LO_SCALE, (x1 - hf.y) * TC_LO_SCALE);
}

int make_tmap(CUtensorMap* tm, const float* base, uint64_t inner, uint64_t mid, uint64_t seeds, uint64_t mid_stride_elems,
              uint64_t seed_stride_elems, uint32_t box_mid);
int launch_gemm(int a_mn, int b_mn, int epi, const CUtensorMap* t, const GemmShape& gs, const EpiParams& ep, cudaStream_t st,
                int kernel_id = -1);
int make_tmap16(CUtensorMap* tm, const void* base, uint64_t inner, uint64_t mid, uint64_t seeds, uint64_t mid_stride_elems,
                uint64_t seed_stride_elems, uint32_t box_mid);
int launch_gemm16(int a_mn, int b_mn, int epi, const CUtensorMap* t, const GemmShape& gs, const EpiParams& ep,
                  cudaStream_t st, int kernel_id = -1);

}
}
```

Measured before the change: 33.53 million.

## Fuse conv+LayerNorm producer into the fp16 wgmma dense GEMM forward

Adds a fused forward kernel in which producer warps build im2col patches from the packed binary observations, run the conv with mma.sync, apply LayerNorm and ReLU, and split the result into fp16 hi/lo tiles written straight into the GEMM's shared-memory A stages. Consumer warps run the existing wgmma dense layer with its LN/head epilogue. This removes the global-memory round trip of the conv activations and one kernel launch per forward. The cost is more complex warp specialisation with register reallocation, and the conv work is recomputed inside each GEMM tile's producer.

```diff
diff --git a/include/pqn_b200.h b/include/pqn_b200.h
--- a/include/pqn_b200.h
+++ b/include/pqn_b200.h
@@ -164,6 +164,7 @@
 
 int pqn_set_tensor_core_path(int on);
 int pqn_set_conv_mma_path(int on);
+int pqn_set_fused_forward(int on);
 
 int pqn_tc_split_lo(const float* x, float* lo, int64_t n, void* stream);
 int pqn_tc_gemm_test(const float* a, const float* a_lo, const float* b, const float* b_lo, float* d, int32_t S,
diff --git a/purejaxql_b200/_lib.py b/purejaxql_b200/_lib.py
--- a/purejaxql_b200/_lib.py
+++ b/purejaxql_b200/_lib.py
@@ -93,6 +93,7 @@
     "pqn_bn_stats_update": (c_int, [c_void_p, c_void_p, c_int32, c_int32, c_int64, c_float, c_float, c_void_p]),
     "pqn_set_tensor_core_path": (c_int, [c_int]),
     "pqn_set_conv_mma_path": (c_int, [c_int]),
+    "pqn_set_fused_forward": (c_int, [c_int]),
     "pqn_tc_split_lo": (c_int, [c_void_p, c_void_p, c_int64, c_void_p]),
     "pqn_tc_split16": (c_int, [c_void_p, c_void_p, c_void_p, c_int64, c_float, c_void_p]),
     "pqn_tc_gemm_test": (c_int, [c_void_p, c_void_p, c_void_p, c_void_p, c_void_p, c_int32, c_int32, c_int32,
diff --git a/purejaxql_b200/csrc/conv16.cuh b/purejaxql_b200/csrc/conv16.cuh
--- /dev/null
+++ b/purejaxql_b200/csrc/conv16.cuh
@@ -0,0 +1,215 @@
+#pragma once
+#include <cuda_fp16.h>
+#include <stdint.h>
+
+#include "../../include/pqn_b200.h"
+#include "tc_common.cuh"
+
+namespace pqn {
+
+constexpr float LN_EPS = 1e-6f;
+constexpr int CONV_O = 16;
+constexpr int CONV_PIX = 64;
+constexpr int FLAT_CNN = CONV_PIX * CONV_O;
+
+template <int C>
+struct ConvCfg {
+  static constexpr int TAPS = 9 * C;
+  static constexpr int OBS_BITS = 100 * C;
+  static constexpr int OBS_WORDS = (OBS_BITS + 31) / 32;
+  static constexpr int PW = (OBS_WORDS + 3) / 4 * 4;
+  static constexpr int SW = PW + 1;
+};
+
+template <int C>
+struct PatchCfg {
+  static constexpr int WORDS = (9 * C + 31) / 32;
+};
+
+template <int C>
+__device__ __forceinline__ void patch_bits(const uint32_t* __restrict__ so, int pix, uint32_t (&w)[PatchCfg<C>::WORDS]) {
+  constexpr int W = PatchCfg<C>::WORDS;
+#pragma unroll
+  for (int k = 0; k < W; ++k) w[k] = 0u;
+  const int y = pix >> 3, x = pix & 7;
+#pragma unroll
+  for (int di = 0; di < 3; ++di) {
+    const int f0 = ((y + di) * 10 + x) * C;
+    const uint32_t r = __funnelshift_r(so[f0 >> 5], so[(f0 >> 5) + 1], f0 & 31) & ((1u << (3 * C)) - 1u);
+    const int o = 3 * C * di;
+    w[o >> 5] |= r << (o & 31);
+    if ((o & 31) + 3 * C > 32) w[min((o >> 5) + 1, W - 1)] |= r >> (32 - (o & 31));
+  }
+}
+
+__device__ __forceinline__ void ln16_quad(const float (&z)[2][4], float& mean0, float& rstd0, float& mean1,
+                                          float& rstd1) {
+  float s0 = z[0][0] + z[0][1] + z[1][0] + z[1][1];
+  float q0 = z[0][0] * z[0][0] + z[0][1] * z[0][1] + z[1][0] * z[1][0] + z[1][1] * z[1][1];
+  float s1 = z[0][2] + z[0][3] + z[1][2] + z[1][3];
+  float q1 = z[0][2] * z[0][2] + z[0][3] * z[0][3] + z[1][2] * z[1][2] + z[1][3] * z[1][3];
+#pragma unroll
+  for (int o = 1; o <= 2; o <<= 1) {
+    s0 += __shfl_xor_sync(0xffffffffu, s0, o); q0 += __shfl_xor_sync(0xffffffffu, q0, o);
+    s1 += __shfl_xor_sync(0xffffffffu, s1, o); q1 += __shfl_xor_sync(0xffffffffu, q1, o);
+  }
+  mean0 = s0 * (1.0f / CONV_O); mean1 = s1 * (1.0f / CONV_O);
+  rstd0 = rsqrtf(fmaxf(q0 * (1.0f / CONV_O) - mean0 * mean0, 0.f) + LN_EPS);
+  rstd1 = rsqrtf(fmaxf(q1 * (1.0f / CONV_O) - mean1 * mean1, 0.f) + LN_EPS);
+}
+
+__device__ __forceinline__ void mma_f16_16n8k16(float (&d)[4], const uint32_t (&a)[4], uint32_t b0, uint32_t b1) {
+  asm volatile(
+      "mma.sync.aligned.m16n8k16.row.col.f32.f16.f16.f32 {%0,%1,%2,%3}, {%4,%5,%6,%7}, {%8,%9}, {%0,%1,%2,%3};"
+      : "+f"(d[0]), "+f"(d[1]), "+f"(d[2]), "+f"(d[3])
+      : "r"(a[0]), "r"(a[1]), "r"(a[2]), "r"(a[3]), "r"(b0), "r"(b1));
+}
+
+template <int C>
+struct Conv16 {
+  static constexpr int TAPS = 9 * C;
+  static constexpr int KS = (TAPS + 15) / 16;
+  static constexpr int ROW = 2 * KS < 8 ? 8 : 2 * KS;
+};
+
+__host__ __device__ constexpr int conv16_channel(int h, int n) { return 4 * (n >> 1) + 2 * h + (n & 1); }
+
+__host__ __device__ constexpr int conv16_tap(int s, int kk) {
+  return 16 * s + (kk < 8 ? 0 : 8) + ((kk & 1) ? 4 : 0) + ((kk & 7) >> 1);
+}
+
+template <int C>
+__device__ __forceinline__ void conv16_load_weights(const float* __restrict__ prm, const pqn_net_layout_t& L, uint4* wb,
+                                                    float* cb, float* sc, float* bi, int tid, int nthr) {
+  using M = Conv16<C>;
+  const float inv255 = 1.0f / 255.0f;
+  for (int i = tid; i < M::KS * 2 * 32; i += nthr) {
+    const int ln = i & 31, h = (i >> 5) & 1, s = i >> 6;
+    const int gg = ln >> 2, tt = ln & 3;
+    const int o = conv16_channel(h, gg);
+    const float scale = __uint_as_float((uint32_t)(127 + 15 - (1 << tt)) << 23);
+    float v[4];
+#pragma unroll
+    for (int q = 0; q < 4; ++q) {
+      const int tap = conv16_tap(s, 2 * tt + (q & 1) + (q >> 1) * 8);
+      v[q] = tap < M::TAPS ? __ldg(prm + L.conv_w + tap * CONV_O + o) * inv255 * scale : 0.f;
+      v[q] = fminf(fmaxf(v[q], -65000.f), 65000.f);
+    }
+    const __half2 h0 = __floats2half2_rn(v[0], v[1]), h1 = __floats2half2_rn(v[2], v[3]);
+    const float2 f0 = __half22float2(h0), f1 = __half22float2(h1);
+    const __half2 l0 = __floats2half2_rn(v[0] - f0.x, v[1] - f0.y), l1 = __floats2half2_rn(v[2] - f1.x, v[3] - f1.y);
+    wb[i] = make_uint4(*reinterpret_cast<const uint32_t*>(&h0), *reinterpret_cast<const uint32_t*>(&h1),
+                       *reinterpret_cast<const uint32_t*>(&l0), *reinterpret_cast<const uint32_t*>(&l1));
+  }
+  if (tid < CONV_O) {
+    cb[tid] = __ldg(prm + L.conv_b + tid);
+    sc[tid] = __ldg(prm + L.ln0_scale + tid);
+    bi[tid] = __ldg(prm + L.ln0_bias + tid);
+  }
+}
+
+template <int C>
+__device__ __forceinline__ void build_patch16(const uint32_t* __restrict__ so, int pix, uint32_t* __restrict__ out) {
+  constexpr int W = PatchCfg<C>::WORDS;
+  uint32_t w[W];
+  patch_bits<C>(so, pix, w);
+#pragma unroll
+  for (int b = 0; b < 2 * Conv16<C>::KS; ++b) {
+    const int o = 8 * b;
+    uint32_t v = (o >> 5) < W ? w[(o >> 5) < W ? (o >> 5) : 0] : 0u;
+    const int sh = o & 31;
+    const uint32_t lo = sh >= 10 ? v >> (sh - 10) : v << (10 - sh);
+    const uint32_t hi = sh + 4 <= 26 ? v << (26 - sh - 4) : v >> (sh + 4 - 26);
+    out[b] = __byte_perm(lo, hi, 0x7610);
+  }
+}
+
+template <int C>
+__device__ __forceinline__ void store_patch16(const uint32_t* __restrict__ so, int pix, uint32_t* __restrict__ row) {
+  using M = Conv16<C>;
+  uint32_t w[M::ROW];
+#pragma unroll
+  for (int k = 0; k < M::ROW; ++k) w[k] = 0u;
+  build_patch16<C>(so, pix, w);
+#pragma unroll
+  for (int q = 0; q < M::ROW / 4; ++q)
+    *reinterpret_cast<uint4*>(row + 4 * q) = make_uint4(w[4 * q], w[4 * q + 1], w[4 * q + 2], w[4 * q + 3]);
+}
+
+template <int C, int NI = 2>
+__device__ __forceinline__ void conv16_block2(const uint32_t* __restrict__ xp, const uint4* __restrict__ wb,
+                                              const float* __restrict__ cb, int mbp, int lane, float (&z)[NI][2][4]) {
+  using M = Conv16<C>;
+  const int g = lane >> 2, t = lane & 3;
+  const uint32_t mask = (1u << (10 + t)) | (1u << (26 + t));
+#pragma unroll
+  for (int i = 0; i < NI; ++i)
+#pragma unroll
+    for (int h = 0; h < 2; ++h) {
+      z[i][h][0] = z[i][h][2] = cb[4 * t + 2 * h];
+      z[i][h][1] = z[i][h][3] = cb[4 * t + 2 * h + 1];
+    }
+  const uint32_t* r00 = xp + (32 * mbp + g) * M::ROW;
+#pragma unroll
+  for (int s = 0; s < M::KS; ++s) {
+    uint32_t a[NI][4];
+#pragma unroll
+    for (int i = 0; i < NI; ++i) {
+      const uint2 w0 = *reinterpret_cast<const uint2*>(r00 + (16 * i) * M::ROW + 2 * s);
+      const uint2 w1 = *reinterpret_cast<const uint2*>(r00 + (16 * i + 8) * M::ROW + 2 * s);
+      a[i][0] = w0.x & mask; a[i][1] = w1.x & mask; a[i][2] = w0.y & mask; a[i][3] = w1.y & mask;
+    }
+    uint4 b[2];
+#pragma unroll
+    for (int h = 0; h < 2; ++h) b[h] = wb[(s * 2 + h) * 32 + lane];
+#pragma unroll
+    for (int h = 0; h < 2; ++h)
+#pragma unroll
+      for (int i = 0; i < NI; ++i) mma_f16_16n8k16(z[i][h], a[i], b[h].z, b[h].w);
+#pragma unroll
+    for (int h = 0; h < 2; ++h)
+#pragma unroll
+      for (int i = 0; i < NI; ++i) mma_f16_16n8k16(z[i][h], a[i], b[h].x, b[h].y);
+  }
+}
+
+__device__ __forceinline__ uint32_t cvt_f16x2_satfinite(float lo, float hi) {
+  uint32_t r;
+  asm("cvt.rn.satfinite.f16x2.f32 %0, %1, %2;" : "=r"(r) : "f"(hi), "f"(lo));
+  return r;
+}
+
+__device__ __forceinline__ void conv16_ln_relu(const float (&z)[2][4], const float* __restrict__ sc,
+                                               const float* __restrict__ bi, int t, float (&x0)[4], float (&x1)[4],
+                                               float (&v0)[4], float (&v1)[4], float& rstd0, float& rstd1) {
+  float mean0, mean1;
+  ln16_quad(z, mean0, rstd0, mean1, rstd1);
+  const float nm0 = -mean0 * rstd0, nm1 = -mean1 * rstd1;
+  const int o4 = 4 * t;
+#pragma unroll
+  for (int h = 0; h < 2; ++h) {
+#pragma unroll
+    for (int c = 0; c < 2; ++c) {
+      const int o = o4 + 2 * h + c;
+      x0[2 * h + c] = fmaf(z[h][c], rstd0, nm0);
+      x1[2 * h + c] = fmaf(z[h][2 + c], rstd1, nm1);
+      v0[2 * h + c] = fmaxf(fmaf(x0[2 * h + c], sc[o], bi[o]), 0.f);
+      v1[2 * h + c] = fmaxf(fmaf(x1[2 * h + c], sc[o], bi[o]), 0.f);
+    }
+  }
+}
+
+__device__ __forceinline__ void conv16_split4(const float (&v)[4], uint2& hi, uint2& lo) {
+  uint32_t hw[2], lw[2];
+#pragma unroll
+  for (int h = 0; h < 2; ++h) {
+    hw[h] = cvt_f16x2_satfinite(v[2 * h], v[2 * h + 1]);
+    const float2 f = __half22float2(*reinterpret_cast<const __half2*>(&hw[h]));
+    const __half2 l = __floats2half2_rn((v[2 * h] - f.x) * tc::TC_LO_SCALE, (v[2 * h + 1] - f.y) * tc::TC_LO_SCALE);
+    lw[h] = *reinterpret_cast<const uint32_t*>(&l);
+  }
+  hi = make_uint2(hw[0], hw[1]);
+  lo = make_uint2(lw[0], lw[1]);
+}
+
+}
diff --git a/purejaxql_b200/csrc/pqn_net.cu b/purejaxql_b200/csrc/pqn_net.cu
--- a/purejaxql_b200/csrc/pqn_net.cu
+++ b/purejaxql_b200/csrc/pqn_net.cu
@@ -4,19 +4,17 @@
 #include "../../include/pqn_b200.h"
 #include "api_common.h"
 #include "tc_common.cuh"
+#include "conv16.cuh"
 
 namespace pqn {
 
 constexpr int GT = 256;
 constexpr int BK = 16;
-constexpr float LN_EPS = 1e-6f;
-constexpr int CONV_O = 16;
-constexpr int CONV_PIX = 64;
 constexpr int HID_CNN = 128;
-constexpr int FLAT_CNN = CONV_PIX * CONV_O;
 
 static int g_use_tc = 2;
 static int g_conv_mma = 1;
+static int g_fused_fwd = 1;
 
 __host__ __device__ static inline int64_t align4(int64_t x) { return (x + 3) & ~(int64_t)3; }
 
@@ -677,14 +675,6 @@
   else qsa_sum[seed] += v;
 }
 
-template <int C>
-struct ConvCfg {
-  static constexpr int TAPS = 9 * C;
-  static constexpr int OBS_BITS = 100 * C;
-  static constexpr int OBS_WORDS = (OBS_BITS + 31) / 32;
-  static constexpr int PW = (OBS_WORDS + 3) / 4 * 4;
-  static constexpr int SW = PW + 1;
-};
 
 template <int C>
 __device__ __forceinline__ uint32_t pixel_bits(const uint32_t* __restrict__ so, int p) {
@@ -972,27 +962,6 @@
 };
 
 template <int C>
-struct PatchCfg {
-  static constexpr int WORDS = (9 * C + 31) / 32;
-};
-
-template <int C>
-__device__ __forceinline__ void patch_bits(const uint32_t* __restrict__ so, int pix, uint32_t (&w)[PatchCfg<C>::WORDS]) {
-  constexpr int W = PatchCfg<C>::WORDS;
-#pragma unroll
-  for (int k = 0; k < W; ++k) w[k] = 0u;
-  const int y = pix >> 3, x = pix & 7;
-#pragma unroll
-  for (int di = 0; di < 3; ++di) {
-    const int f0 = ((y + di) * 10 + x) * C;
-    const uint32_t r = __funnelshift_r(so[f0 >> 5], so[(f0 >> 5) + 1], f0 & 31) & ((1u << (3 * C)) - 1u);
-    const int o = 3 * C * di;
-    w[o >> 5] |= r << (o & 31);
-    if ((o & 31) + 3 * C > 32) w[min((o >> 5) + 1, W - 1)] |= r >> (32 - (o & 31));
-  }
-}
-
-template <int C>
 __device__ __forceinline__ void build_patch(const uint32_t* __restrict__ so, int pix, uint32_t* __restrict__ out) {
   constexpr int W = PatchCfg<C>::WORDS;
   uint32_t w[W];
@@ -1091,22 +1060,6 @@
 #pragma unroll
       for (int i = 0; i < 2; ++i) mma_tf32_16n8k8(z[i][h], a[i], __float_as_uint(bh[h].x), __float_as_uint(bh[h].y));
   }
-}
-
-__device__ __forceinline__ void ln16_quad(const float (&z)[2][4], float& mean0, float& rstd0, float& mean1,
-                                          float& rstd1) {
-  float s0 = z[0][0] + z[0][1] + z[1][0] + z[1][1];
-  float q0 = z[0][0] * z[0][0] + z[0][1] * z[0][1] + z[1][0] * z[1][0] + z[1][1] * z[1][1];
-  float s1 = z[0][2] + z[0][3] + z[1][2] + z[1][3];
-  float q1 = z[0][2] * z[0][2] + z[0][3] * z[0][3] + z[1][2] * z[1][2] + z[1][3] * z[1][3];
-#pragma unroll
-  for (int o = 1; o <= 2; o <<= 1) {
-    s0 += __shfl_xor_sync(0xffffffffu, s0, o); q0 += __shfl_xor_sync(0xffffffffu, q0, o);
-    s1 += __shfl_xor_sync(0xffffffffu, s1, o); q1 += __shfl_xor_sync(0xffffffffu, q1, o);
-  }
-  mean0 = s0 * (1.0f / CONV_O); mean1 = s1 * (1.0f / CONV_O);
-  rstd0 = rsqrtf(fmaxf(q0 * (1.0f / CONV_O) - mean0 * mean0, 0.f) + LN_EPS);
-  rstd1 = rsqrtf(fmaxf(q1 * (1.0f / CONV_O) - mean1 * mean1, 0.f) + LN_EPS);
 }
 
 constexpr int CONV_MMA_WARPS = 8;
@@ -1245,127 +1198,6 @@
   }
 }
 
-__device__ __forceinline__ void mma_f16_16n8k16(float (&d)[4], const uint32_t (&a)[4], uint32_t b0, uint32_t b1) {
-  asm volatile(
-      "mma.sync.aligned.m16n8k16.row.col.f32.f16.f16.f32 {%0,%1,%2,%3}, {%4,%5,%6,%7}, {%8,%9}, {%0,%1,%2,%3};"
-      : "+f"(d[0]), "+f"(d[1]), "+f"(d[2]), "+f"(d[3])
-      : "r"(a[0]), "r"(a[1]), "r"(a[2]), "r"(a[3]), "r"(b0), "r"(b1));
-}
-
-template <int C>
-struct Conv16 {
-  static constexpr int TAPS = 9 * C;
-  static constexpr int KS = (TAPS + 15) / 16;
-  static constexpr int ROW = 2 * KS < 8 ? 8 : 2 * KS;
-};
-
-__host__ __device__ constexpr int conv16_channel(int h, int n) { return 4 * (n >> 1) + 2 * h + (n & 1); }
-
-__host__ __device__ constexpr int conv16_tap(int s, int kk) {
-  return 16 * s + (kk < 8 ? 0 : 8) + ((kk & 1) ? 4 : 0) + ((kk & 7) >> 1);
-}
-
-template <int C>
-__device__ __forceinline__ void conv16_load_weights(const float* __restrict__ prm, const pqn_net_layout_t& L, uint4* wb,
-                                                    float* cb, float* sc, float* bi) {
-  using M = Conv16<C>;
-  const float inv255 = 1.0f / 255.0f;
-  for (int i = threadIdx.x; i < M::KS * 2 * 32; i += blockDim.x) {
-    const int ln = i & 31, h = (i >> 5) & 1, s = i >> 6;
-    const int gg = ln >> 2, tt = ln & 3;
-    const int o = conv16_channel(h, gg);
-    const float scale = __uint_as_float((uint32_t)(127 + 15 - (1 << tt)) << 23);
-    float v[4];
-#pragma unroll
-    for (int q = 0; q < 4; ++q) {
-      const int tap = conv16_tap(s, 2 * tt + (q & 1) + (q >> 1) * 8);
-      v[q] = tap < M::TAPS ? __ldg(prm + L.conv_w + tap * CONV_O + o) * inv255 * scale : 0.f;
-      v[q] = fminf(fmaxf(v[q], -65000.f), 65000.f);
-    }
-    const __half2 h0 = __floats2half2_rn(v[0], v[1]), h1 = __floats2half2_rn(v[2], v[3]);
-    const float2 f0 = __half22float2(h0), f1 = __half22float2(h1);
-    const __half2 l0 = __floats2half2_rn(v[0] - f0.x, v[1] - f0.y), l1 = __floats2half2_rn(v[2] - f1.x, v[3] - f1.y);
-    wb[i] = make_uint4(*reinterpret_cast<const uint32_t*>(&h0), *reinterpret_cast<const uint32_t*>(&h1),
-                       *reinterpret_cast<const uint32_t*>(&l0), *reinterpret_cast<const uint32_t*>(&l1));
-  }
-  if (threadIdx.x < CONV_O) {
-    cb[threadIdx.x] = __ldg(prm + L.conv_b + threadIdx.x);
-    sc[threadIdx.x] = __ldg(prm + L.ln0_scale + threadIdx.x);
-    bi[threadIdx.x] = __ldg(prm + L.ln0_bias + threadIdx.x);
-  }
-}
-
-template <int C>
-__device__ __forceinline__ void build_patch16(const uint32_t* __restrict__ so, int pix, uint32_t* __restrict__ out) {
-  constexpr int W = PatchCfg<C>::WORDS;
-  uint32_t w[W];
-  patch_bits<C>(so, pix, w);
-#pragma unroll
-  for (int b = 0; b < 2 * Conv16<C>::KS; ++b) {
-    const int o = 8 * b;
-    uint32_t v = (o >> 5) < W ? w[(o >> 5) < W ? (o >> 5) : 0] : 0u;
-    const int sh = o & 31;
-    const uint32_t lo = sh >= 10 ? v >> (sh - 10) : v << (10 - sh);
-    const uint32_t hi = sh + 4 <= 26 ? v << (26 - sh - 4) : v >> (sh + 4 - 26);
-    out[b] = __byte_perm(lo, hi, 0x7610);
-  }
-}
-
-template <int C>
-__device__ __forceinline__ void store_patch16(const uint32_t* __restrict__ so, int pix, uint32_t* __restrict__ row) {
-  using M = Conv16<C>;
-  uint32_t w[M::ROW];
-#pragma unroll
-  for (int k = 0; k < M::ROW; ++k) w[k] = 0u;
-  build_patch16<C>(so, pix, w);
-#pragma unroll
-  for (int q = 0; q < M::ROW / 4; ++q)
-    *reinterpret_cast<uint4*>(row + 4 * q) = make_uint4(w[4 * q], w[4 * q + 1], w[4 * q + 2], w[4 * q + 3]);
-}
-
-template <int C>
-__device__ __forceinline__ void conv16_block2(const uint32_t* __restrict__ xp, const uint4* __restrict__ wb,
-                                              const float* __restrict__ cb, int mbp, int lane, float (&z)[2][2][4]) {
-  using M = Conv16<C>;
-  const int g = lane >> 2, t = lane & 3;
-  const uint32_t mask = (1u << (10 + t)) | (1u << (26 + t));
-#pragma unroll
-  for (int i = 0; i < 2; ++i)
-#pragma unroll
-    for (int h = 0; h < 2; ++h) {
-      z[i][h][0] = z[i][h][2] = cb[4 * t + 2 * h];
-      z[i][h][1] = z[i][h][3] = cb[4 * t + 2 * h + 1];
-    }
-  const uint32_t* r00 = xp + (32 * mbp + g) * M::ROW;
-#pragma unroll
-  for (int s = 0; s < M::KS; ++s) {
-    uint32_t a[2][4];
-#pragma unroll
-    for (int i = 0; i < 2; ++i) {
-      const uint2 w0 = *reinterpret_cast<const uint2*>(r00 + (16 * i) * M::ROW + 2 * s);
-      const uint2 w1 = *reinterpret_cast<const uint2*>(r00 + (16 * i + 8) * M::ROW + 2 * s);
-      a[i][0] = w0.x & mask; a[i][1] = w1.x & mask; a[i][2] = w0.y & mask; a[i][3] = w1.y & mask;
-    }
-    uint4 b[2];
-#pragma unroll
-    for (int h = 0; h < 2; ++h) b[h] = wb[(s * 2 + h) * 32 + lane];
-#pragma unroll
-    for (int h = 0; h < 2; ++h)
-#pragma unroll
-      for (int i = 0; i < 2; ++i) mma_f16_16n8k16(z[i][h], a[i], b[h].z, b[h].w);
-#pragma unroll
-    for (int h = 0; h < 2; ++h)
-#pragma unroll
-      for (int i = 0; i < 2; ++i) mma_f16_16n8k16(z[i][h], a[i], b[h].x, b[h].y);
-  }
-}
-
-__device__ __forceinline__ uint32_t cvt_f16x2_satfinite(float lo, float hi) {
-  uint32_t r;
-  asm("cvt.rn.satfinite.f16x2.f32 %0, %1, %2;" : "=r"(r) : "f"(hi), "f"(lo));
-  return r;
-}
-
 constexpr int CONV16_WARPS = 4;
 constexpr int CONV16_CTAS_PER_SM = 5;
 
@@ -1385,7 +1217,7 @@
   const int tid = threadIdx.x, warp = tid >> 5, lane = tid & 31;
   const int g = lane >> 2, t = lane & 3;
   const int seed = blockIdx.y;
-  conv16_load_weights<C>(params + (int64_t)seed * P, L, wb, cb, sc, bi);
+  conv16_load_weights<C>(params + (int64_t)seed * P, L, wb, cb, sc, bi, threadIdx.x, blockDim.x);
   if (TRAIN && tid < C) s_cnt[tid] = 0.f;
   __syncthreads();
   int cnt[C];
@@ -2474,11 +2306,14 @@
 }
 
 static int tc16_dense_fwd(int epi, const float* params, int64_t P, const pqn_net_layout_t& L, const Workspace& w,
-                          const Planes16& pl, int A, float* q, int S, int rows, cudaStream_t st) {
+                          const Planes16& pl, int A, float* q, int S, int rows, cudaStream_t st,
+                          const tc::ConvIn* ci = nullptr, int C = 0) {
   CUtensorMap t[4];
   int rc;
-  if ((rc = tc::make_tmap16(&t[0], pl.h1_hi, FLAT_CNN, rows, S, FLAT_CNN, (uint64_t)rows * FLAT_CNN, 128))) return rc;
-  if ((rc = tc::make_tmap16(&t[1], pl.h1_lo, FLAT_CNN, rows, S, FLAT_CNN, (uint64_t)rows * FLAT_CNN, 128))) return rc;
+  if (!ci) {
+    if ((rc = tc::make_tmap16(&t[0], pl.h1_hi, FLAT_CNN, rows, S, FLAT_CNN, (uint64_t)rows * FLAT_CNN, 128))) return rc;
+    if ((rc = tc::make_tmap16(&t[1], pl.h1_lo, FLAT_CNN, rows, S, FLAT_CNN, (uint64_t)rows * FLAT_CNN, 128))) return rc;
+  }
   if ((rc = tc::make_tmap16(&t[2], pl.w1_hi, HID_CNN, FLAT_CNN, S, HID_CNN, (uint64_t)FLAT_CNN * HID_CNN, 64))) return rc;
   if ((rc = tc::make_tmap16(&t[3], pl.w1_lo, HID_CNN, FLAT_CNN, S, HID_CNN, (uint64_t)FLAT_CNN * HID_CNN, 64))) return rc;
   tc::GemmShape gs = {};
@@ -2487,6 +2322,7 @@
   ep.params = params; ep.P = P; ep.off_b = L.d0_b; ep.off_scale = L.ln1_scale; ep.off_bias = L.ln1_bias;
   ep.off_hw = L.head_w; ep.off_hb = L.head_b; ep.A = A; ep.rows = rows;
   ep.H = w.h2; ep.XHAT = w.xhat2; ep.RSTD = w.rstd2; ep.Q = q;
+  if (ci) return tc::launch_conv_gemm16(C, t + 2, gs, ep, *ci, st, K_TC_FWD_HEAD);
   return tc::launch_gemm16(0, 1, epi, t, gs, ep, st, epi == tc::EPI_LN_HEAD ? K_TC_FWD_HEAD : K_TC_FWD);
 }
 
@@ -2877,6 +2713,12 @@
   return PQN_OK;
 }
 
+int pqn_set_fused_forward(int on) {
+  if (on != 0 && on != 1) return set_error(PQN_E_UNSUPPORTED, "pqn_set_fused_forward: no forward path %d", on);
+  g_fused_fwd = on;
+  return PQN_OK;
+}
+
 int pqn_set_tensor_core_path(int on) {
   if (on < 0 || on > 2) return set_error(PQN_E_UNSUPPORTED, "pqn_set_tensor_core_path: no tensor-core path %d", on);
   g_use_tc = on;
@@ -2937,6 +2779,13 @@
     const bool f16 = use_tc && g_use_tc == 2;
     const Planes16 pl = planes16(w, S, rows);
     const bool conv16 = f16 && g_conv_mma == 1;
+    if (conv16 && g_fused_fwd) {
+      launch_split16_w1(params, L.total, L.d0_w, pl, S, st);
+      const tc::ConvIn ci = {(const uint32_t*)obs, obs_rows_per_seed, gather, params, L.total, L};
+      if ((rc = tc16_dense_fwd(tc::EPI_LN_HEAD, params, L.total, L, w, pl, A, q, S, (int)rows, st, &ci, d->in_c)))
+        return rc;
+      return check_launch("pqn_qnet_forward");
+    }
     launch_conv_fwd<false>(d->in_c, dim3(cdiv(rows, 4), S), st, (const uint32_t*)obs, obs_rows_per_seed, gather, params,
                            L.total, L, conv16 ? (float*)pl.h1_hi : w.h1, conv16 ? (float*)pl.h1_lo : nullptr, nullptr,
                            (int)rows, nullptr, nullptr, nullptr, conv16);
diff --git a/purejaxql_b200/csrc/pqn_tc.cu b/purejaxql_b200/csrc/pqn_tc.cu
--- a/purejaxql_b200/csrc/pqn_tc.cu
+++ b/purejaxql_b200/csrc/pqn_tc.cu
@@ -5,6 +5,7 @@
 #include "../../include/pqn_b200.h"
 #include "api_common.h"
 #include "tc_common.cuh"
+#include "conv16.cuh"
 
 namespace pqn {
 namespace tc {
@@ -231,11 +232,131 @@
 
 __device__ __forceinline__ void wg_bar_sync(int wg) { asm volatile("bar.sync %0, 128;" ::"r"(3 + wg) : "memory"); }
 
-template <int A_MN, int B_MN, int EPI, bool F16 = true>
-__global__ void __launch_bounds__(TC_THREADS, 1)
+template <int R>
+__device__ __forceinline__ void setmaxnreg_inc() { asm volatile("setmaxnreg.inc.sync.aligned.u32 %0;" ::"n"(R)); }
+template <int R>
+__device__ __forceinline__ void setmaxnreg_dec() { asm volatile("setmaxnreg.dec.sync.aligned.u32 %0;" ::"n"(R)); }
+__device__ __forceinline__ void producer_bar_sync(int nthreads) {
+  asm volatile("bar.sync 5, %0;" ::"r"(nthreads) : "memory");
+}
+
+template <int C>
+struct ConvTile {
+  using M = Conv16<C>;
+  static constexpr int NI = M::ROW == 8 ? 2 : 1;
+  static constexpr int NPW = NI == 2 ? 8 : 4;
+  static constexpr int THREADS = TC_CONSUMERS + 32 * NPW;
+  static constexpr int LAUNCH_REGS = (65536 / THREADS) & ~7;
+  static constexpr int REG_PRODUCER = NPW == 8 ? 88 : 96;
+  static constexpr int REG_CONSUMER = NPW == 8 ? 168 : 200;
+  static_assert(TC_CONSUMERS * REG_CONSUMER + 32 * NPW * REG_PRODUCER <= THREADS * LAUNCH_REGS,
+                "setmaxnreg redistributes the CTA's launch allocation");
+  static constexpr int RW = 128 / NPW;
+  static constexpr int SPS = RW < 16 * NI ? RW : 16 * NI;
+  static constexpr int PPS = 16 * NI / SPS;
+  static constexpr int PW = ConvCfg<C>::PW;
+  static constexpr int SW = ConvCfg<C>::SW;
+  static_assert(SW % 2 == 1, "conflict-free observation rows");
+  static constexpr int WB_BYTES = M::KS * 2 * 32 * 16;
+  static constexpr int PATCH_WORDS = 16 * NI * M::ROW;
+  static constexpr int SMEM_BYTES = TC_SMEM_BYTES + WB_BYTES + NPW * PATCH_WORDS * 4 + 3 * CONV_O * 4 + 128 * SW * 4;
+  static_assert(SMEM_BYTES <= 227 * 1024, "dynamic shared memory of the fused forward exceeds the per-CTA limit");
+};
+
+template <int C>
+__device__ __forceinline__ void conv_producer(uint8_t* smem_al, uint32_t smem_base, uint64_t* full, uint64_t* empty,
+                                              uint8_t* conv_smem, const CUtensorMap* tm_b_hi,
+                                              const CUtensorMap* tm_b_lo, const GemmShape& gs, const ConvIn& ci) {
+  using M = Conv16<C>;
+  using T = ConvTile<C>;
+  constexpr int NI = T::NI, SPS = T::SPS, PPS = T::PPS, SGROUPS = T::RW / SPS;
+  uint4* wb = reinterpret_cast<uint4*>(conv_smem);
+  uint32_t* patch_all = reinterpret_cast<uint32_t*>(conv_smem + T::WB_BYTES);
+  float* cb = reinterpret_cast<float*>(patch_all + T::NPW * T::PATCH_WORDS);
+  float* sc = cb + CONV_O;
+  float* bi = sc + CONV_O;
+  uint32_t* so_all = reinterpret_cast<uint32_t*>(bi + CONV_O);
+  const int pt = threadIdx.x - TC_CONSUMERS, pw = pt >> 5, lane = pt & 31;
+  const int g = lane >> 2, t = lane & 3;
+  uint32_t* patch = patch_all + pw * T::PATCH_WORDS;
+  uint32_t* so = so_all + pw * T::RW * T::SW;
+  const int num_tiles = gs.m_tiles * gs.S;
+  int stage = 0, cur_seed = -1;
+  uint32_t phase = 0;
+  for (int tile = blockIdx.x; tile < num_tiles; tile += gridDim.x) {
+    const int seed = tile / gs.m_tiles;
+    const int m0 = (tile - seed * gs.m_tiles) * 128;
+    if (seed != cur_seed) {
+      producer_bar_sync(32 * T::NPW);
+      conv16_load_weights<C>(ci.params + (int64_t)seed * ci.P, ci.L, wb, cb, sc, bi, pt, 32 * T::NPW);
+      producer_bar_sync(32 * T::NPW);
+      cur_seed = seed;
+    }
+    __syncwarp();
+    for (int i = lane; i < T::RW * T::PW; i += 32) {
+      const int r = i / T::PW, wd = i - r * T::PW, m = m0 + T::RW * pw + r;
+      uint32_t v = 0u;
+      if (m < gs.M) {
+        const int64_t src = ci.gather ? __ldg(ci.gather + (int64_t)seed * gs.M + m) : m;
+        v = __ldg(ci.obs + ((int64_t)seed * ci.obs_rows_per_seed + src) * T::PW + wd);
+      }
+      so[r * T::SW + wd] = v;
+    }
+    for (int kb = 0; kb < gs.k_blocks; ++kb) {
+      mbar_wait(&empty[stage], phase ^ 1u);
+      if (pt == 0) {
+        const uint32_t sb = smem_base + stage * TC_STAGE_BYTES;
+        mbar_expect_tx(&full[stage], 2 * TC_TILE_BYTES);
+#pragma unroll
+        for (int j = 0; j < 2; ++j) {
+          tma_load_3d(sb + TC_B_HI + j * 8192, tm_b_hi, &full[stage], 64 * j, kb * TC_BK16, seed);
+          tma_load_3d(sb + TC_B_LO + j * 8192, tm_b_lo, &full[stage], 64 * j, kb * TC_BK16, seed);
+        }
+      }
+      uint8_t* a_hi = smem_al + stage * TC_STAGE_BYTES + TC_A_HI;
+      uint8_t* a_lo = smem_al + stage * TC_STAGE_BYTES + TC_A_LO;
+#pragma unroll 1
+      for (int step = 0; step < SGROUPS * 4 / PPS; ++step) {
+        const int j0 = (step / SGROUPS) * PPS, r0 = (step % SGROUPS) * SPS;
+        __syncwarp();
+        if (lane < 16 * NI)
+          store_patch16<C>(so + (r0 + lane % SPS) * T::SW, 4 * kb + j0 + lane / SPS, patch + lane * M::ROW);
+        __syncwarp();
+        float z[NI][2][4];
+        conv16_block2<C, NI>(patch, wb, cb, 0, lane, z);
+#pragma unroll
+        for (int i = 0; i < NI; ++i) {
+          float x0[4], x1[4], v0[4], v1[4], rs0, rs1;
+          conv16_ln_relu(z[i], sc, bi, t, x0, x1, v0, v1, rs0, rs1);
+          uint2 h0, l0, h1, l1;
+          conv16_split4(v0, h0, l0);
+          conv16_split4(v1, h1, l1);
+          const int ra = T::RW * pw + r0 + (16 * i + g) % SPS, rb = ra + 8;
+          const int j = j0 + (16 * i) / SPS;
+          const int off = ((((2 * j + (t >> 1)) ^ g)) << 4) | ((t & 1) << 3);
+          const uint2 zero = make_uint2(0u, 0u);
+          const bool oka = m0 + ra < gs.M, okb = m0 + rb < gs.M;
+          *reinterpret_cast<uint2*>(a_hi + ra * 128 + off) = oka ? h0 : zero;
+          *reinterpret_cast<uint2*>(a_lo + ra * 128 + off) = oka ? l0 : zero;
+          *reinterpret_cast<uint2*>(a_hi + rb * 128 + off) = okb ? h1 : zero;
+          *reinterpret_cast<uint2*>(a_lo + rb * 128 + off) = okb ? l1 : zero;
+        }
+      }
+      fence_proxy_async_smem();
+      __syncwarp();
+      if (lane == 0) mbar_arrive(&full[stage]);
+      if (++stage == TC_STAGES) { stage = 0; phase ^= 1u; }
+    }
+  }
+}
+
+template <int A_MN, int B_MN, int EPI, bool F16 = true, int CONVC = 0>
+__global__ void __launch_bounds__(CONVC ? ConvTile<CONVC ? CONVC : 4>::THREADS : TC_THREADS, 1)
     tc_gemm_kernel(const __grid_constant__ CUtensorMap tm_a_hi, const __grid_constant__ CUtensorMap tm_a_lo,
                    const __grid_constant__ CUtensorMap tm_b_hi, const __grid_constant__ CUtensorMap tm_b_lo,
-                   const __grid_constant__ CUtensorMap tm_out, const GemmShape gs, const EpiParams ep) {
+                   const __grid_constant__ CUtensorMap tm_out, const GemmShape gs, const EpiParams ep,
+                   const ConvIn ci) {
+  static_assert(!CONVC || (A_MN == 0 && B_MN == 1 && EPI == EPI_LN_HEAD && F16), "the fused forward's layout");
   constexpr bool TMA_EPI = tma_store_epilogue<EPI, F16>();
   extern __shared__ __align__(1024) uint8_t smem_raw[];
   const uint32_t smem_base = (smem_u32(smem_raw) + 1023u) & ~1023u;
@@ -248,12 +369,24 @@
   const int warp = threadIdx.x >> 5, lane = threadIdx.x & 31;
 
   if (warp == 8 && lane == 0) {
-    prefetch_tmap(&tm_a_hi); prefetch_tmap(&tm_a_lo); prefetch_tmap(&tm_b_hi); prefetch_tmap(&tm_b_lo);
+    if (!CONVC) { prefetch_tmap(&tm_a_hi); prefetch_tmap(&tm_a_lo); }
+    prefetch_tmap(&tm_b_hi); prefetch_tmap(&tm_b_lo);
     if (TMA_EPI) prefetch_tmap(&tm_out);
-    for (int i = 0; i < TC_STAGES; ++i) { mbar_init(&full[i], 1); mbar_init(&empty[i], TC_CONSUMERS / 32); }
+    for (int i = 0; i < TC_STAGES; ++i) {
+      mbar_init(&full[i], 1 + (CONVC ? ConvTile<CONVC ? CONVC : 4>::NPW : 0));
+      mbar_init(&empty[i], TC_CONSUMERS / 32);
+    }
     fence_barrier_init();
   }
   __syncthreads();
+  if constexpr (CONVC != 0) {
+    if (warp >= 8) {
+      setmaxnreg_dec<ConvTile<CONVC>::REG_PRODUCER>();
+      conv_producer<CONVC>(smem_al, smem_base, full, empty, reinterpret_cast<uint8_t*>(full) + 256, &tm_b_hi, &tm_b_lo, gs, ci);
+      return;
+    }
+    setmaxnreg_inc<ConvTile<CONVC>::REG_CONSUMER>();
+  }
 
   const int ksplit = gs.k_split > 1 ? gs.k_split : 1;
   const int kb_per = (gs.k_blocks + ksplit - 1) / ksplit;
@@ -536,11 +669,13 @@
   return PQN_OK;
 }
 
-template <int A_MN, int B_MN, int EPI, bool F16>
-static int launch_t(const CUtensorMap* t, const GemmShape& gs, const EpiParams& ep, cudaStream_t st, int kid) {
-  auto kfn = tc_gemm_kernel<A_MN, B_MN, EPI, F16>;
+template <int A_MN, int B_MN, int EPI, bool F16, int CONVC = 0>
+static int launch_t(const CUtensorMap* t, const GemmShape& gs, const EpiParams& ep, cudaStream_t st, int kid,
+                    const ConvIn& ci = ConvIn{}) {
+  auto kfn = tc_gemm_kernel<A_MN, B_MN, EPI, F16, CONVC>;
   static_assert(TC_SMEM_BYTES <= 227 * 1024, "dynamic shared memory of the GEMM kernel exceeds the per-CTA limit");
-  if (cudaFuncSetAttribute(kfn, cudaFuncAttributeMaxDynamicSharedMemorySize, TC_SMEM_BYTES) != cudaSuccess)
+  constexpr int smem = CONVC ? ConvTile<CONVC ? CONVC : 4>::SMEM_BYTES : TC_SMEM_BYTES;
+  if (cudaFuncSetAttribute(kfn, cudaFuncAttributeMaxDynamicSharedMemorySize, smem) != cudaSuccess)
     return check_launch("tc_gemm(cudaFuncSetAttribute)");
   CUtensorMap tm_out = t[0];
   if (tma_store_epilogue<EPI, F16>()) {
@@ -554,7 +689,7 @@
   const int grid = tiles < num_sms() ? tiles : num_sms();
   {
     LaunchScope _ls(kid < 0 ? (int)K_TC_GEMM : kid, st);
-    kfn<<<grid, TC_THREADS, TC_SMEM_BYTES, st>>>(t[0], t[1], t[2], t[3], tm_out, gs, ep);
+    kfn<<<grid, CONVC ? ConvTile<CONVC ? CONVC : 4>::THREADS : TC_THREADS, smem, st>>>(t[0], t[1], t[2], t[3], tm_out, gs, ep, ci);
   }
   return check_launch("tc_gemm");
 }
@@ -587,6 +722,20 @@
   PQN_TC_CASE(0, 0, EPI_RELU_BITS)
 #undef PQN_TC_CASE
   return set_error(PQN_E_UNSUPPORTED, "tc_gemm16: combination a_mn=%d b_mn=%d epi=%d not instantiated", a_mn, b_mn, epi);
+}
+
+int launch_conv_gemm16(int C, const CUtensorMap* tb, const GemmShape& gs, const EpiParams& ep, const ConvIn& ci,
+                       cudaStream_t st, int kernel_id) {
+  if (gs.n_tiles != 1 || gs.k_split > 1 || gs.k_blocks != FLAT_CNN / TC_BK16)
+    return set_error(PQN_E_INVALID, "tc_conv_gemm16: the fused forward is 1024 x 128 without split-K");
+  const CUtensorMap t[4] = {tb[0], tb[1], tb[0], tb[1]};
+  switch (C) {
+    case 4: return launch_t<0, 1, EPI_LN_HEAD, true, 4>(t, gs, ep, st, kernel_id, ci);
+    case 6: return launch_t<0, 1, EPI_LN_HEAD, true, 6>(t, gs, ep, st, kernel_id, ci);
+    case 7: return launch_t<0, 1, EPI_LN_HEAD, true, 7>(t, gs, ep, st, kernel_id, ci);
+    case 10: return launch_t<0, 1, EPI_LN_HEAD, true, 10>(t, gs, ep, st, kernel_id, ci);
+  }
+  return set_error(PQN_E_UNSUPPORTED, "tc_conv_gemm16: no fused forward for %d input channels", C);
 }
 
 int make_tmap16(CUtensorMap* tm, const void* base, uint64_t inner, uint64_t mid, uint64_t seeds, uint64_t mid_stride_elems,
diff --git a/purejaxql_b200/csrc/tc_common.cuh b/purejaxql_b200/csrc/tc_common.cuh
--- a/purejaxql_b200/csrc/tc_common.cuh
+++ b/purejaxql_b200/csrc/tc_common.cuh
@@ -2,6 +2,8 @@
 #include <cuda.h>
 #include <cuda_fp16.h>
 #include <stdint.h>
+
+#include "../../include/pqn_b200.h"
 
 namespace pqn {
 namespace tc {
@@ -47,6 +49,15 @@
   int64_t P, off_b, off_scale, off_bias, off_hw, off_hb;
   int A, rows;
   float *H, *XHAT, *RSTD, *Q;
+};
+
+struct ConvIn {
+  const uint32_t* obs;
+  int64_t obs_rows_per_seed;
+  const int32_t* gather;
+  const float* params;
+  int64_t P;
+  pqn_net_layout_t L;
 };
 
 __device__ __forceinline__ uint32_t smem_u32(const void* p) { return (uint32_t)__cvta_generic_to_shared(p); }
@@ -161,6 +172,8 @@
                 uint64_t seed_stride_elems, uint32_t box_mid);
 int launch_gemm16(int a_mn, int b_mn, int epi, const CUtensorMap* t, const GemmShape& gs, const EpiParams& ep,
                   cudaStream_t st, int kernel_id = -1);
+int launch_conv_gemm16(int C, const CUtensorMap* tb, const GemmShape& gs, const EpiParams& ep, const ConvIn& ci,
+                       cudaStream_t st, int kernel_id = -1);
 
 }
 }
```

After: 34.16 million, median of 6. 1.02x the previous value.
